# raphiniert-com/volume_renderer

Hardware: AMD Instinct MI355X
Metric: Mrays/s + achieved HBM GB/s, 1024³ vol @ 1920×1080 HG-shaded, 1/2/4/8 GPU (higher is better)
Workload: dtype f32; 1 GPU; V_shell(1024) fp32 1024^3, 1920x1080, HG 2 lights (example1.m), on-the-fly gradient, rotate(125,25,0) f=3 dist=6 thr=0.9; lights=2, gradient=compute, parallelism=image-column partition x1 (block 16), depth_lanes=2, frames=serial, one HIP stream

## Files before the change

volume_renderer_amd/csrc/vr_capi.hip:

```cpp
#include <hip/hip_runtime.h>

#include <algorithm>
#include <chrono>
#include <cmath>
#include <cstdio>
#include <cstdlib>
#include <cstring>
#include <memory>
#include <mutex>
#include <map>
#include <set>
#include <array>
#include <sstream>
#include <string>
#include <queue>
#include <vector>

#include "../../include/vrhip.h"
#include "vr_device.h"
#include "vr_resources.h"
#include "vr_transfer.h"

#ifndef VR_WITH_K8
#define VR_WITH_K8 0
// ... 361 lines not shown
  if (!want || b->occ_bytes != bytes) {
    if (b->occ) vr_host::pooled_free(b->occ, b->occ_bytes, b->device, vr_host::Readers(b->readers));
    b->occ = nullptr;
    b->occ_bytes = 0;
  }
  if (!want) return;
  if (!b->occ) {
    VR_HIP(vr_host::pooled_alloc(reinterpret_cast<void **>(&b->occ), bytes, b->device));
    b->occ_bytes = bytes;
  }
  const float inv = (!b->nonfinite && b->maxabs > 0.f) ? 255.f / b->maxabs : 0.f;
  VR_HIP(vr::launch_occupancy(b->ptr, (uint32_t)px, (uint32_t)py, (uint32_t)pz, b->occ, std::isfinite(inv) ? inv : 0.f,
                              s));
  VR_HIP(hipStreamSynchronize(s));
}

void sync_volume(vr_context *h, int tex, int slot) {
  g_tex.bind[tex].reset();
  const VolRec &v = h->vol[slot];
  const uint64_t n = v.dims[0] * v.dims[1] * v.dims[2];
  const uint64_t padded = n ? (v.dims[0] + 2) * (v.dims[1] + 2) * (v.dims[2] + 2) * sizeof(float) : 0;
  BufPtr b = h->buf[slot];
  if (!(b && b.use_count() == 2 && b->bytes == padded && b->device == h->device && b->readers.done())) {
    h->buf[slot].reset();
    b = std::make_shared<DevBuf>();
    b->device = h->device;
    b->bytes = padded;
    if (padded) VR_HIP(vr_host::pooled_alloc(reinterpret_cast<void **>(&b->ptr), padded, h->device));
  }
  for (int i = 0; i < 3; ++i) b->dims[i] = v.dims[i];
  b->nonfinite = false;
  b->maxabs = 0.f;
  b->readers.clear();
  if (n) {
    if (!v.data) throw HipError{hipErrorInvalidValue, "volume data is NULL"};
    vr_host::Uploader &U = vr_host::uploaders()[h->device];
    VR_HIP(U.init(h->device));
    vr::BufStats st{0u, 0.f};
    VR_HIP(U.upload(v.data, v.dtype, v.location == VR_DEVICE, (int32_t)v.dims[0], (int32_t)v.dims[1],
                    (int32_t)v.dims[2], b->ptr, &st));
    b->nonfinite = st.nonfinite != 0;
    b->maxabs = st.maxabs;
    if (tex == T_LIGHT) build_zpair(b.get(), U.stream);
    else if (tex <= T_RE) build_occupancy(b.get(), U.stream);
  } else {
    build_occupancy(b.get(), nullptr);
  }
  b->version = next_version();
  b->src_data = v.data;
  b->src_last_update = v.last_update;
  b->src_bytes = v.memory_size;
  b->src_dtype = v.dtype;
  h->buf[slot] = b;
  g_tex.bind[tex] = b;
}

void sync_volume_if_changed(vr_context *h, int tex, int slot) {
  const BufPtr &b = g_tex.bind[tex];
  const VolRec &v = h->vol[slot];
  if (b && h->buf[slot] == b && b->device == h->device && v.data && b->src_data == v.data &&
      b->src_last_update == v.last_update && b->src_bytes == v.memory_size && b->src_dtype == v.dtype &&
      v.last_update != 0 &&
      !env_flag("VR_ALWAYS_REUPLOAD"))
    return;
  sync_volume(h, tex, slot);
}

template <class S>
void sync_decisions(S &s, bool simEmAb, bool simEmRe, bool simAbRe, bool reqEm, bool reqAb, bool reqRe) {
  bool updEm = false, updAb = false, updRe = false;
  if (reqEm) {
    if (!updEm) { s.upload(T_EM); updEm = true; }
    if (simEmRe && !updRe) { s.reference(T_RE, T_RE, &S::idx_re, T_EM); updRe = true; }
    if (simEmAb && !updAb) { s.reference(T_AB, T_AB, &S::idx_ab, T_EM); updAb = true; }
  }
  if (reqAb) {
    if (!updAb) { s.upload(T_AB); updAb = true; }
    if (simAbRe && !updRe) { s.reference(T_RE, T_RE, &S::idx_re, T_AB); updRe = true; }
    if (simEmAb && !updEm) { s.reference(T_EM, T_AB, &S::idx_em, T_AB); updEm = true; }
  }
  if (reqRe) {
    if (!updRe) { s.upload(T_RE); updRe = true; }
    if (simAbRe && !updAb) { s.reference(T_AB, T_AB, &S::idx_ab, T_RE); updAb = true; }
    if (simEmAb && !updEm) { s.reference(T_EM, T_EM, &S::idx_em, T_RE); updEm = true; }
  }
}

struct RealState {
  vr_context *h;
  int32_t idx_em, idx_ab, idx_re;
  void upload(int slot) { sync_volume(h, slot, slot); }
  void reference(int tex, int bufslot, int32_t RealState::*idx, int target) {
    if (h->buf[bufslot]) {
      g_tex.bind[tex].reset();
      h->buf[bufslot].reset();
    }
    this->*idx = target;
  }
};

struct DebugState {
  bool present[3] = {true, true, true};
  bool bound[3] = {true, true, true};
  int32_t idx_em, idx_ab, idx_re;
  void upload(int slot) { present[slot] = true; bound[slot] = true; }
  void reference(int tex, int bufslot, int32_t DebugState::*idx, int target) {
    if (present[bufslot]) {
      bound[tex] = false;
      present[bufslot] = false;
    }
    this->*idx = target;
  }
};

uint64_t required_memory(const vr_context *h) {
  const VolRec &em = h->vol[T_EM], &ab = h->vol[T_AB], &re = h->vol[T_RE];
  uint64_t r = em.memory_size;
  if (!same(em, ab) && !same(re, ab)) r += ab.memory_size;
  if (!same(em, re) && !same(re, ab)) r += re.memory_size;
  r += h->vol[T_DX].memory_size + h->vol[T_DY].memory_size + h->vol[T_DZ].memory_size;
  return r;
}

int check_free_device_memory(uint64_t required) {
  size_t free_b = 0, total_b = 0;
  VR_HIP(hipMemGetInfo(&free_b, &total_b));
  if (free_b >= required) return VR_OK;
  int dev = 0;
  VR_HIP(hipGetDevice(&dev));
  vr_host::pool_clear(dev);
  vr_host::prune_retired(true);
  VR_HIP(hipMemGetInfo(&free_b, &total_b));
  if (free_b >= required) return VR_OK;
  std::ostringstream os;
  os << "insufficient free VRAM!\n"
     << "\tTotal Memory (MB): \t" << total_b / (1024 * 1024) << "\n"
     << "\tFree Memory (MB): \t" << free_b / (1024 * 1024) << "\n"
     << "\tRequired memory (MB): \t" << required / (1024 * 1024) << "\n";
  return fail(VR_ERR_VRAM, os.str());
}

void reset_gradients(vr_context *h) {
  for (int s : {T_DX, T_DY, T_DZ}) {
    h->buf[s].reset();
    h->vol[s] = VolRec();
  }
}

void mm_sync(vr_context *h) {
  if ((h->vol[T_DX].last_update == 0 && h->buf[T_DX]) || (h->vol[T_DY].last_update == 0 && h->buf[T_DY]) ||
      (h->vol[T_DZ].last_update == 0 && h->buf[T_DZ]))
    reset_gradients(h);
  const VolRec &em = h->vol[T_EM], &ab = h->vol[T_AB], &re = h->vol[T_RE];
  const uint64_t T = h->time_last_mem_sync;
  RealState s{h, g_tex.idx_em, g_tex.idx_ab, g_tex.idx_re};
  sync_decisions(s, same(em, ab), same(em, re), same(ab, re), em.last_update > T || T == 0,
                 ab.last_update > T || T == 0, re.last_update > T || T == 0);
  g_tex.idx_em = s.idx_em;
  g_tex.idx_ab = s.idx_ab;
  g_tex.idx_re = s.idx_re;
  if (h->vol[T_DX].last_update != 0 && h->vol[T_DY].last_update != 0 && h->vol[T_DZ].last_update != 0) {
    sync_volume_if_changed(h, T_DX, T_DX);
    sync_volume_if_changed(h, T_DY, T_DY);
    sync_volume_if_changed(h, T_DZ, T_DZ);
    g_tex.grad_method = G_LOOKUP;
  }
}

vr::DevTex dev_tex(const BufPtr &b) {
  vr::DevTex t{};
  if (b && b->ptr) {
    t.p = b->ptr;
    t.nx = (int32_t)b->dims[0];
    t.ny = (int32_t)b->dims[1];
    t.nz = (int32_t)b->dims[2];
    t.px = (uint32_t)(b->dims[0] + 2);
    t.pxy = (uint32_t)((b->dims[0] + 2) * (b->dims[1] + 2));
    t.fnx = (float)t.nx;
    t.fny = (float)t.ny;
    t.fnz = (float)t.nz;
    t.one = (t.nx == 1 && t.ny == 1 && t.nz == 1);
    const uint64_t padded = (b->dims[0] + 2) * (b->dims[1] + 2) * (b->dims[2] + 2);
    t.small = padded < (1ull << 22) && !test_flag("VR_NO_SMALL_LUT");
    t.fpx4 = 4.f * (float)t.px;
    t.fpxy4 = 4.f * (float)t.pxy;
    t.fbase4 = 4.f * (float)(t.pxy + t.px + 1);
    t.zp = t.small ? b->zpair : nullptr;
  }
  return t;
}

bool is_big(const vr::DevTex &t) {
  return t.p && ((uint64_t)t.nx + 2) * ((uint64_t)t.ny + 2) * ((uint64_t)t.nz + 2) > 0xFFFFFFFFull;
}

bool same_tex(const vr::DevTex &a, const vr::DevTex &b) {
  return a.p == b.p && a.nx == b.nx && a.ny == b.ny && a.nz == b.nz;
}
bool same_dims(const vr::DevTex &a, const vr::DevTex &b) {
  return a.nx == b.nx && a.ny == b.ny && a.nz == b.nz;
}

bool tame(const BufPtr &b) { return !b || !b->ptr || (!b->nonfinite && b->maxabs < 1e30f); }

int32_t half_texel_taps(const vr::RenderParams &P, int mode, float fnz) {
  if (mode != 1 || test_flag("VR_EXACT_TAPS")) return 0;
  const float n[3] = {P.em.fnx, P.em.fny, fnz};
  for (int i = 0; i < 3; ++i) {
    int e = 0;
    if (!(n[i] >= 2.f) || std::frexp(n[i], &e) != 0.5f) return 0;
    if (P.gstep[i] != 1.f / n[i] || P.bscale[i] != 0.5f || P.bmin[i] != -1.f) return 0;
  }
  return 1;
}

struct Frame {
  vr::RenderParams P;
  double drift1[3] = {0, 0, 0};
  int mode = 0;
  bool ab_alias = false, big = false, share = false;
  bool degenerate = false;
  vr_context::Schedule *sched_copy = nullptr;
  vr_context::Schedule *sched = nullptr;
};


void drift_bound(Frame &F, const float *eye2) {
  const vr::RenderParams &P = F.P;
  double pmax = 0.0;
  for (int i = 0; i < 3; ++i) {
    double e = std::fabs(P.eye[i]);
    if (eye2) e = std::max(e, (double)std::fabs(eye2[i]));
    pmax = std::max(pmax, (double)std::fabs(P.bmin[i]) + e);
  }
  for (int i = 0; i < 3; ++i) {
    const float n = i == 0 ? P.em.fnx : (i == 1 ? P.em.fny : P.em.fnz);
    F.drift1[i] = 2.0 * pmax * 1.2e-7 * (double)P.bscale[i] * (double)n;
    F.P.probe_off[i] = (float)(0.0625 + (double)VR_PROBE_MAX * F.drift1[i]);
  }
}

int build_frame(vr_context *h, const vr_render_args *a, Frame &F, uint64_t depth_override = 0) {
  vr::RenderParams &P = F.P;
  std::memset(&P, 0, sizeof(P));
  const uint64_t H = a->resolution[0], W = a->resolution[1];
  if (W > 0x7FFFFFFF || H > 0x7FFFFFFF || W * H > (1ull << 40))
    return fail(VR_ERR_UNSUPPORTED, "image resolution too large");
  P.width = (int32_t)W;
  P.height = (int32_t)H;
  P.fw = (float)W;
  P.fh = (float)H;
  P.ratio = (float)H / (float)W;
  P.fe = a->factors[0];
  P.fr = a->factors[1];
  P.fa = a->factors[2];
  const float es[3] = {a->element_size_um[2], a->element_size_um[1], a->element_size_um[0]};
  const VolRec &ev = h->vol[T_EM];
  const uint64_t vw = ev.dims[0], vh = ev.dims[1], vd = depth_override ? depth_override : ev.dims[2];
  float bmax[3];
  bmax[0] = 1.f;
  bmax[1] = (es[1] * (float)vh) / ((float)vw * es[0]);
  bmax[2] = (es[2] * (float)vd) / ((float)vw * es[0]);
  for (int i = 0; i < 3; ++i) P.bmin[i] = -1.f * bmax[i];
  const float dxy = sqrtf((float)(vw * vw + vh * vh));
  const float dyz = sqrtf((float)(vh * vh + vd * vd));
  const float dxz = sqrtf((float)(vw * vw + vd * vd));
  const float mind = fminf(dxy, fminf(dyz, dxz));
  P.tstep = 1.f / (2.2f * mind);
  P.thr = a->opacity_threshold;
  for (int i = 0; i < 3; ++i) {
    P.bscale[i] = 1.f / (bmax[i] - P.bmin[i]);
    P.color[i] = a->color[i];
  }
  P.gstep[0] = 1.f / (float)vw;
  P.gstep[1] = 1.f / (float)vh;
  P.gstep[2] = 1.f / (float)vd;
  const float *r = a->rotation_flipped;
  const float X[3] = {r[2], r[1], r[0]}, Y[3] = {r[5], r[4], r[3]}, Z[3] = {r[8], r[7], r[6]};
  const float xoff = a->props[0], f = a->props[1], dist = a->props[2];
  for (int i = 0; i < 3; ++i) {
    P.eye[i] = fmaf(-dist, Z[i], xoff * X[i]);
    P.ydir[i] = Y[i];
    P.zdir[i] = Z[i];
  }
  const float xx = fmaf(X[2], X[2], fmaf(X[1], X[1], X[0] * X[0]));
  const float xinv = 1.f / sqrtf(xx);
  for (int i = 0; i < 3; ++i) P.nx_[i] = X[i] * xinv;
  P.focal = f;
  P.em = dev_tex(g_tex.bind[g_tex.idx_em]);
  {
    const BufPtr &eb = g_tex.bind[g_tex.idx_em];
    P.occ = (eb && eb->ptr && eb->occ) ? eb->occ : nullptr;
    constexpr uint64_t E = 1u << VR_OCC_LOG;
    P.occ_bx = P.occ ? (uint32_t)((eb->dims[0] + 2 + E - 1) / E) : 0u;
    P.occ_bxy = P.occ ? P.occ_bx * (uint32_t)((eb->dims[1] + 2 + E - 1) / E) : 0u;
  }
  P.ab = dev_tex(g_tex.bind[g_tex.idx_ab]);
  P.re = dev_tex(g_tex.bind[g_tex.idx_re]);
  P.gem = dev_tex(g_tex.bind[T_EM]);
  P.gx = dev_tex(g_tex.bind[T_DX]);
  P.gy = dev_tex(g_tex.bind[T_DY]);
  P.gz = dev_tex(g_tex.bind[T_DZ]);
  P.lut = dev_tex(g_tex.bind[T_LIGHT]);
  P.num_lights = (int32_t)g_tex.lights.size();
  P.lights = nullptr;
  F.mode = P.num_lights == 0 ? 0 : (g_tex.grad_method == G_LOOKUP ? 2 : 1);
  F.ab_alias = same_tex(P.ab, P.em);
  const bool em_grid = P.em.p && !P.em.one;
  if (F.mode == 1)
    F.share = em_grid && same_tex(P.gem, P.em);
  else if (F.mode == 2)
    F.share = em_grid && P.gx.p && P.gy.p && P.gz.p && !P.gx.one && same_dims(P.gx, P.em) &&
              same_dims(P.gy, P.em) && same_dims(P.gz, P.em);
  P.re_is_em = same_tex(P.re, P.em) && P.em.p != nullptr;
  {
    drift_bound(F, nullptr);
    for (int i = 0; i < 3; ++i) {
      const float n = i == 0 ? P.em.fnx : (i == 1 ? P.em.fny : P.em.fnz);
      P.tap_off[i] = (float)((F.mode == 1 ? (double)P.gstep[i] * P.bscale[i] * n : 0.0) + 0.0625);
    }
    P.tap_half = half_texel_taps(P, F.mode, P.em.fnz);
    P.cube_hs[0] = P.tap_half ? P.em.fnx * 0.5f : 0.f;
    P.cube_hs[1] = P.tap_half ? P.em.fny * 0.5f : 0.f;
    P.cube_hs[2] = P.tap_half ? P.em.fnz * 0.5f : 0.f;
  }
  {
    const BufPtr &rb = g_tex.bind[g_tex.idx_re];
    const BufPtr &lb = g_tex.bind[T_LIGHT];
    bool ok = tame(rb) && tame(lb) && std::isfinite(P.fr) && std::fabs(P.fr) < 1e3f;
    double bound = 1.0;
    for (int i = 0; i < 3; ++i) {
      ok = ok && std::isfinite(P.color[i]) && std::fabs(P.color[i]) < 1e3f;
      bound = std::max(bound, (double)std::fabs(P.color[i]));
    }
    double lmax = 0.0;
    for (const auto &L : g_tex.lights) {
      for (float c : {L.cr, L.cg, L.cb}) {
        ok = ok && std::isfinite(c);
        lmax = std::max(lmax, (double)std::fabs(c));
      }
    }
    const double rmax = (rb && rb->ptr) ? rb->maxabs : 0.0, lutmax = (lb && lb->ptr) ? lb->maxabs : 0.0;
    ok = ok && (double)std::fabs(P.fr) * rmax * lutmax * lmax * bound * (double)(g_tex.lights.size() + 1) < 1e36;
    P.skip_empty = ok ? 1 : 0;
    if (const char *ev = test_env("VR_NO_EMPTY_SKIP"))
      if (ev[0] == '1') P.skip_empty = 0;
    if (P.skip_empty && test_flag("VR_NO_BRICK_TEST")) P.skip_empty = 2;
  }
  {
    const BufPtr &eb = g_tex.bind[g_tex.idx_em], &ab = g_tex.bind[g_tex.idx_ab];
    auto vmax = [](const BufPtr &b) { return (b && b->ptr) ? (b->nonfinite ? INFINITY : (double)b->maxabs) : 0.0; };
    const double xa = std::fabs((double)P.fa) * vmax(ab) * (double)P.tstep;
    const double xe = std::fabs((double)P.fe) * vmax(eb) * (double)P.tstep;
    P.small_x = (std::isfinite(xa) && xa < 0x1p-7 * 0.999) ? 1 : 0;
    P.eds_finite = (std::isfinite(xe) && xe < 1e38) ? 1 : 0;
    if (diag_flag("VR_NO_RANGE_FLAGS")) P.small_x = P.eds_finite = 0;
  }
  {
    const bool re_ok = P.re_is_em || (P.re.p && P.re.one);
    const bool lut_ok = g_tex.lights.empty() || (P.lut.p && P.lut.small && !P.lut.one && P.lut.zp &&
                                                 std::max(P.lut.nx, std::max(P.lut.ny, P.lut.nz)) <= 8192);
    const bool step_ok = std::isfinite(P.tstep) && P.tstep > 0.f;
    P.tame = (P.skip_empty && P.eds_finite && P.small_x && re_ok && lut_ok && step_ok && !diag_flag("VR_NO_TAME")) ? 1
                                                                                                            : 0;
    P.re_mask = P.re_is_em ? 0xffffffffu : 0u;
  }
  F.big = is_big(P.em) || is_big(P.ab) || is_big(P.re) || is_big(P.gem) || is_big(P.gx) || is_big(P.gy) ||
          is_big(P.gz) || test_flag("VR_FORCE_BIG");
  if (F.mode == 2 && P.gx.p &&
      vr::interleave3_entries(P.gx.px, P.gx.pxy / P.gx.px, (uint32_t)P.gx.nz + 2u) > 0xFFFFFFFFull)
    F.big = true;
  if (is_big(P.lut)) return fail(VR_ERR_UNSUPPORTED, "illumination volume larger than 2^32 voxels");
  bool finite = std::isfinite(P.tstep) && P.tstep > 0.f;
  for (int i = 0; i < 3; ++i) finite = finite && std::isfinite(P.bmin[i]) && std::isfinite(P.bscale[i]);
  const double diag = std::sqrt(4.0 * ((double)bmax[0] * bmax[0] + (double)bmax[1] * bmax[1] +
                                       (double)bmax[2] * bmax[2]));
  const double cap = 2.0 * diag / (double)P.tstep + 64.0;
  P.max_steps = (finite && cap < 2.0e9) ? (int32_t)cap : 2000000000;
  F.degenerate = !finite;
  return VR_OK;
}

void upload_lights(vr_context *h, const vr_render_args *a) {
  if (a->num_lights < 0 || !a->illumination) return;
  const size_t n = (size_t)a->num_lights;
  g_tex.lights.resize(n);
  for (size_t l = 0; l < n; ++l) {
    const vr_light &L = a->lights[l];
    g_tex.lights[l] = vr::DevLight{L.position[2], L.position[1], L.position[0], L.color[0], L.color[1],
                                   L.color[2]};
  }
  h->vol[T_LIGHT] = make_rec(a->illumination);
  sync_volume_if_changed(h, T_LIGHT, T_LIGHT);
}

using LaunchRec = vr_host::LaunchRec<BufPtr>;
void wait_ready(const BufPtr &b, hipStream_t s) {
  if (b && !vr_host::done(b->ready)) VR_HIP(hipStreamWaitEvent(s, b->ready->e, 0));
}
void bind_reads(LaunchRec &L) {
  for (const BufPtr &b : g_tex.bind)
    if (b) {
      wait_ready(b, L.stream);
      L.reads.push_back(b);
    }
  for (const auto &kv : g_tex.gvec)
    if (kv.second.buf && kv.first == L.device) {
      wait_ready(kv.second.buf, L.stream);
      L.reads.push_back(kv.second.buf);
    }
}
void stage_frame(LaunchRec &L, vr::RenderParams &P, const std::vector<vr::DevLight> &lights) {
  const void *d = nullptr;
  VR_HIP(L.stage(lights.data(), lights.size() * sizeof(vr::DevLight), &d));
  P.lights = static_cast<const vr::DevLight *>(d);
}

int64_t part_columns(int64_t w, int32_t bc, int32_t part, int32_t np) {
  if (w <= 0) return 0;
  if (np <= 1) return w;
  const int64_t nblocks = (w + bc - 1) / bc;
  int64_t cols = 0;
  for (int64_t b = part; b < nblocks; b += np) cols += std::min<int64_t>(bc, w - b * bc);
  return cols;
}

int validate_partition(const vr_partition *p) {
  if (!p) return VR_OK;
  if (p->num_parts < 1 || p->part < 0 || p->part >= p->num_parts || p->block_cols < 1)
    return fail(VR_ERR_ARGUMENT, "invalid partition");
  return VR_OK;
}


int chunk_samples(int K) { return K >= 2 ? 16 * K : 32; }
void set_chunk_halo(Frame &F, int K) {
  for (int i = 0; i < 3; ++i) {
    F.P.tap_off[i] += (float)(chunk_samples(K) * F.drift1[i]);
  }
}

void free_views(vr_context *h) {
  if (h->d_chan) (void)hipFree(h->d_chan);
  h->d_chan = nullptr;
  h->d_chan_bytes = 0;
}

void free_schedules(vr_context *h) {
  for (auto &kv : h->sched) {
    if (kv.second.copied) (void)hipEventSynchronize(kv.second.copied);
    if (kv.second.d_cost) (void)hipFree(kv.second.d_cost);
    if (kv.second.d_order) (void)hipFree(kv.second.d_order);
    if (kv.second.h_cost) (void)hipHostFree(kv.second.h_cost);
    if (kv.second.pre_flag) (void)hipFree(kv.second.pre_flag);
    if (kv.second.pre_count) (void)hipFree(kv.second.pre_count);
    if (kv.second.pre_state) (void)hipFree(kv.second.pre_state);
    if (kv.second.copied) (void)hipEventDestroy(kv.second.copied);
  }
  h->sched.clear();
}

int device_wave_slots() {
  static int slots = 0;
  if (!slots) {
    int dev = 0, cus = 256;
    if (hipGetDevice(&dev) == hipSuccess) {
      hipDeviceProp_t prop;
      if (hipGetDeviceProperties(&prop, dev) == hipSuccess && prop.multiProcessorCount > 0)
        cus = prop.multiProcessorCount;
    }
    slots = cus * 16;
  }
  return slots;
}

#ifndef VR_COUNT_K
#define VR_COUNT_K 0
#endif
#ifndef VR_XCD_RUN
#define VR_XCD_RUN 0
#endif

int depth_lanes(const vr::RenderParams &P) {
  if (const char *ev = test_env("VR_DEPTH_LANES")) {
    const int k = std::atoi(ev);
    if (k == 1 || k == 2 || k == 4 || (k == 8 && VR_WITH_K8)) return k;
  }
  const double waves = std::ceil(P.part_cols / 8.0) * std::ceil(P.height / 8.0);
  const double rounds = waves / device_wave_slots();
  const double tau = P.tau > 0.f ? (double)P.tau : 1.0;
  if (P.lookup) return 4;
  if (rounds < VR_DEPTH_ROUNDS_K2 || tau >= VR_DEPTH_TAU_K4) return 4;
  if (rounds >= VR_DEPTH_ROUNDS_K1 && tau < VR_DEPTH_TAU_K1) return 1;
  return 2;
}

void set_tau_and_slot(vr::RenderParams &P, const vr_render_args *a, double vw) {
  const double f = std::fabs((double)a->props[1]), dist = std::fabs((double)a->props[2]);
  const double tau = (f > 0 && P.width > 0) ? dist * vw / ((double)P.width * f) : 1e30;
  P.tau = (float)std::min(tau, 1e30);
  const int K = P.steps ? 1 : depth_lanes(P);
  P.wide_slot = (tau > 1.5 || (K >= 4 && !P.lookup)) ? 1 : 0;
  if (const char *ev = test_env("VR_WIDE_SLOT")) P.wide_slot = std::atoi(ev) ? 1 : 0;
}

bool short_launch(const vr::RenderParams &P) {
  const double rounds = std::ceil(P.part_cols / 8.0) * std::ceil(P.height / 8.0) * std::max(1, (int)P.views) /
                        device_wave_slots();
  return rounds < VR_SCHED_ROUNDS;
}
#ifndef VR_SCHED_LPT_ROUNDS
#define VR_SCHED_LPT_ROUNDS 32.0
#endif
bool lpt_launch(const vr::RenderParams &P) {
  const double rounds = std::ceil(P.part_cols / 8.0) * std::ceil(P.height / 8.0) * std::max(1, (int)P.views) /
                        device_wave_slots();
  return rounds < VR_SCHED_ROUNDS || rounds >= VR_SCHED_LPT_ROUNDS;
}
bool want_schedule(const vr::RenderParams &P) {
  if (P.views > 2 || (P.views == 2 && test_flag("VR_STEREO_PAIR")) || test_flag_off("VR_SCHED")) return false;
  return test_flag("VR_SCHED") || short_launch(P) || !test_flag_off("VR_SCHED_FULL");
}

uint64_t wg_tail_arg(uint32_t tail_pct) {
  return (uint64_t)tail_pct << 32 | (uint64_t)(device_wave_slots() / 16 * 6);
}

uint64_t frame_key(const vr::RenderParams &P) {
  uint64_t h = 1469598103934665603ull;
  auto mix = [&h](const void *p, size_t n) {
    const unsigned char *c = static_cast<const unsigned char *>(p);
    for (size_t i = 0; i < n; ++i) h = (h ^ c[i]) * 1099511628211ull;
  };
  mix(P.eye, sizeof P.eye);
  mix(P.eye2, sizeof P.eye2);
  mix(P.nx_, sizeof P.nx_);
  mix(P.ydir, sizeof P.ydir);
  mix(P.zdir, sizeof P.zdir);
  mix(&P.focal, sizeof P.focal);
  mix(P.bmin, sizeof P.bmin);
  mix(&P.tstep, sizeof P.tstep);
  mix(&P.thr, sizeof P.thr);
  mix(&P.fa, sizeof P.fa);
  mix(&P.fe, sizeof P.fe);
  mix(&P.em.p, sizeof P.em.p);
  mix(&P.occ, sizeof P.occ);
  const BufPtr &eb = g_tex.bind[g_tex.idx_em];
  const uint64_t ver = (eb && eb->ptr == P.em.p) ? eb->version : 0;
  mix(&ver, sizeof ver);
  return h | 1u;
}

#ifndef VR_PRED_STEP_TEXELS
#define VR_PRED_STEP_TEXELS 8.0
#endif
hipError_t predict_costs(const vr::RenderParams &P, int K, uint32_t nb_view, uint32_t *cost, hipStream_t stream) {
  const int TW = K == 1 ? 8 : (K == 2 ? 4 : (K == 4 ? 4 : 2)), TH = K <= 2 ? 8 : 4;
  const uint32_t nbx = (uint32_t)((P.part_cols + 2 * TW - 1) / (2 * TW));
  const BufPtr &eb = g_tex.bind[g_tex.idx_em];
  double dens = 0.0;
  if (eb && !eb->nonfinite && P.fa > 0.f && std::isfinite(P.fa))
    dens = (double)P.fa * (double)eb->maxabs / 255.0 * (double)P.tstep;
  const double xthr = P.thr < 1.f ? -std::log1p(-(double)std::max(P.thr, 0.f)) : 1e30;
  double tpa = 0.0;
  for (int i = 0; i < 3; ++i) {
    const float n = i == 0 ? P.em.fnx : (i == 1 ? P.em.fny : P.em.fnz);
    tpa = std::max(tpa, (double)P.bscale[i] * (double)n);
  }
  const double per = (double)P.tstep * tpa;
  const int m = (int)std::max(1.0, std::min(4096.0, std::floor(VR_PRED_STEP_TEXELS / std::max(per, 1e-9))));
  const hipError_t rc = vr::launch_predict_cost(P, nb_view, nbx, TW, TH, m, (float)dens, (float)std::min(xthr, 1e30),
                                                cost, stream);
  if (const char *dump = rc == hipSuccess ? diag_env("VR_SCHED_PRED_DUMP") : nullptr) {
    const uint32_t nb = nb_view * (uint32_t)std::max(1, (int)P.views);
    std::vector<uint32_t> c(nb);
    VR_HIP(hipMemcpyAsync(c.data(), cost, (size_t)nb * 4, hipMemcpyDeviceToHost, stream));
    VR_HIP(hipStreamSynchronize(stream));
    const uint32_t hdr[4] = {(uint32_t)K, (uint32_t)P.part, (uint32_t)P.num_parts, nb};
    if (FILE *f = std::fopen(dump, "ab")) {
      std::fwrite(hdr, 4, 4, f);
      std::fwrite(c.data(), 4, c.size(), f);
      std::fclose(f);
    }
  }
  return rc;
}

hipError_t attach_schedule(vr_context *h, vr::RenderParams &P, Frame &F, int K, hipStream_t stream,
                           const char *extra) {
  typedef uint32_t (*blocks_fn)(const vr::RenderParams &);
  static const blocks_fn bfns[4] = {vr::fast::march_blocks_k1, vr::fast::march_blocks_k2, vr::fast::march_blocks_k4,
                                    VR_K8(vr::fast::march_blocks_k8, vr::fast::march_blocks_k4)};
  const int ki = K == 1 ? 0 : K == 2 ? 1 : K == 4 ? 2 : 3;
  const uint32_t nb_view = bfns[ki](P);
  const uint32_t nb = nb_view * (uint32_t)std::max(1, (int)P.views);
  char key[300];
  std::snprintf(key, sizeof key, "%d/%d/%d/%d/%d/%d/%d/%d/%d/%u/%p/%s", K, P.width, P.height, P.part, P.num_parts,
                P.block_cols, F.mode, P.wide_slot, P.fast_shade, nb, (void *)stream, extra);
  vr_context::Schedule &S = h->sched[key];
  F.sched = &S;
  if (!S.d_cost && nb) {
    hipError_t e = hipMalloc(&S.d_cost, nb * sizeof(uint32_t));
    if (e == hipSuccess) e = hipMalloc(&S.d_order, nb * sizeof(uint32_t));
    if (e != hipSuccess) {
      vr_host::consume(e, "hipMalloc (launch schedule; the launch runs unscheduled)");
      if (S.d_cost) (void)hipFree(S.d_cost);
      S.d_cost = nullptr;
      S.d_order = nullptr;
    }
    S.blocks = nb;
  }
  if (!(S.d_cost && S.blocks == nb)) return hipSuccess;
  hipError_t rc = hipSuccess;
  const bool full = !lpt_launch(P) && !test_flag("VR_SCHED");
  const uint64_t fkey = frame_key(P);
  const bool predict = P.occ && P.occ_bx && !diag_flag("VR_SCHED_MEASURED");
  if (!full) {
    P.sched_full = 0;
    if (S.measured && S.key == fkey) {
      rc = vr::launch_order(S.d_cost, nb, S.d_order, stream, 0u, 0u);
    } else if (predict) {
      rc = predict_costs(P, K, nb_view, S.d_cost, stream);
      if (rc == hipSuccess) rc = vr::launch_order(S.d_cost, nb, S.d_order, stream, 0u, 0u);
    } else {
      rc = vr::launch_iota(S.d_order, nb, stream);
    }
    S.measured = true;
    S.key = fkey;
    S.pred_key = 0;
  } else {
    if (S.key != fkey) {
      if (S.copy_pending) {
        (void)hipEventSynchronize(S.copied);
        S.copy_pending = false;
      }
      S.measured = S.decided = S.tail = S.order_stale = false;
      S.frames = S.renders = 0;
      S.key = fkey;
    }
    ++S.renders;
    uint32_t every = VR_SCHED_REMEASURE;
    if (const char *ev = test_env("VR_SCHED_REMEASURE")) every = (uint32_t)std::max(1, std::atoi(ev));
    uint32_t heavy_div = VR_SCHED_HEAVY_DIV;
    if (const char *ev = diag_env("VR_SCHED_HEAVY_DIV")) heavy_div = (uint32_t)std::max(1, std::atoi(ev));
    uint32_t tail_pct = VR_SCHED_TAIL_PCT;
    if (const char *ev = test_env("VR_SCHED_TAIL_PCT")) tail_pct = (uint32_t)std::max(0, std::atoi(ev));
    if (!S.h_cost) {
      hipError_t e = hipHostMalloc(reinterpret_cast<void **>(&S.h_cost), nb * sizeof(uint32_t));
      if (e == hipSuccess) e = hipEventCreateWithFlags(&S.copied, hipEventDisableTiming);
      if (e != hipSuccess) {
        vr_host::consume(e, "hipHostMalloc / hipEventCreate (full-frame schedule; none used)");
        return hipSuccess;
      }
    }
    if (S.copy_pending && vr_host::query_done(S.copied, "hipEventQuery (schedule durations)")) {
      S.copy_pending = false;
      uint64_t sum = 0;
      uint32_t mx = 0;
      for (uint32_t i = 0; i < nb; ++i) {
        sum += S.h_cost[i];
        mx = std::max(mx, S.h_cost[i]);
      }
      const uint64_t wg_slots = std::max<uint64_t>(1, (uint64_t)(device_wave_slots() / 16 * 6));
      S.tail = (uint64_t)mx * 100u >= (sum / wg_slots) * tail_pct;
      S.decided = true;
      S.order_stale = true;
    }
    if (predict && !S.decided) {
      if (S.pred_key != fkey) {
        rc = predict_costs(P, K, nb_view, S.d_cost, stream);
        if (rc == hipSuccess) rc = vr::launch_order(S.d_cost, nb, S.d_order, stream, heavy_div, wg_tail_arg(0));
        S.pred_key = rc == hipSuccess ? fkey : 0;
      }
      if (S.renders >= 2 && !S.measured && !diag_flag("VR_SCHED_PREDICT_ONLY")) {
        S.measured = true;
        S.frames = 0;
        P.sched_full = 1;
        F.sched_copy = &S;
      } else {
        P.sched_full = 2;
      }
// ... 1914 lines not shown
```

volume_renderer_amd/csrc/vr_device.h:

```cpp
#pragma once
#include <stdint.h>
#include <hip/hip_runtime.h>

namespace vr {

struct DevTex {
  const float *p;
  int32_t nx, ny, nz;
  uint32_t px;
  uint32_t pxy;
  float fnx, fny, fnz;
  int32_t one;
  int32_t small;
  float fpx4, fpxy4, fbase4;
  const float *zp;
};

#ifndef VR_PROBE_MAX
#define VR_PROBE_MAX 512
#endif

#ifndef VR_OCC_LOG
#define VR_OCC_LOG 3
#endif

#ifndef VR_GVEC_BRICK
#define VR_GVEC_BRICK 1
#endif

struct DevLight {
  float px, py, pz;
  float cr, cg, cb;
};

struct RenderParams {
  int32_t width, height;
  float fw, fh;
  float ratio;
  float fe, fa, fr;
  float bmin[3];
  float bscale[3];
  float eye[3];
  float eye2[3];
  float nx_[3];
  float ydir[3], zdir[3];
  float focal;
  float thr, tstep;
  int32_t max_steps;
  float color[3];
  float gstep[3];
  float tap_off[3];
  int32_t tap_half;
  float cube_hs[3];
  int32_t num_lights;
  const DevLight *lights;
  DevTex em, ab, re, gem, gx, gy, gz, lut;
  const float *gvec;
  uint32_t gv_row8, gv_plane8;
  int32_t re_is_em;
  int32_t skip_empty;
  int32_t small_x;
  int32_t eds_finite;
  int32_t tame;
  uint32_t re_mask;
  float tau;
  int32_t lookup;
  int32_t tile_mode;
  int32_t xcd_run;
  uint32_t block_rot;
  int32_t wide_slot;
  int32_t fast_shade;
  int32_t block_cols, part, num_parts, part_cols;
  int32_t plane_cols;
  float *out;
  float *out2;
  int32_t views;
  int32_t pair_shift;
  uint32_t view_blocks;
  const uint32_t *wg_order;
  uint32_t *wg_cost;
  uint32_t *wg_start;
  uint32_t sched_blocks;
  uint32_t sched_full;
  uint32_t prio_blocks;
  const uint8_t *occ;
  uint32_t occ_bx, occ_bxy;
  float probe_off[3];
  unsigned long long *steps;
  float slab_z0, slab_z1, slab_margin;
  int32_t slab_pk0, slab_pk1, slab_dir;
  const float *slab_in;
  const uint32_t *pre_flag;
  float4 *pre_state;
  uint32_t *pre_count;
  uint32_t pre_cap;
};

#define VR_VIEWS_MAX 4
struct RenderViews {
  RenderParams p[VR_VIEWS_MAX];
};
static_assert(sizeof(RenderViews) <= 4160, "RenderParams grew: RenderViews passes four by value as kernel arguments");

struct BufStats {
  uint32_t nonfinite;
  float maxabs;
};

void note_march_kernel(bool fast, int K, int mode, bool ab, bool count, bool share, bool big, int cap, int sched,
                       int nl);
bool test_switches_on();

}
```

volume_renderer_amd/csrc/vr_march.hip:

```cpp
#include <hip/hip_runtime.h>
#include <stdint.h>
#include <math.h>
#include <stdlib.h>
#include <algorithm>
#include <type_traits>

#ifndef VR_MARCH_K
#define VR_MARCH_K 1
#endif
#ifndef VR_MERGED_BOUNDS
#define VR_MERGED_BOUNDS 1
#endif
#ifndef VR_WHOLE_BOX
#define VR_WHOLE_BOX 1
#endif
#ifndef VR_CHECK_WHOLE
#define VR_CHECK_WHOLE 0
#endif
#ifndef VR_LIGHTS_HOIST
#define VR_LIGHTS_HOIST 1
#endif
#ifndef VR_REFL_HOIST
#define VR_REFL_HOIST 1
#endif
#ifndef VR_ADAPTIVE_S
#define VR_ADAPTIVE_S 1
#endif
#ifndef VR_WHOLE_SPLIT
#define VR_WHOLE_SPLIT 1
#endif
#ifndef VR_COUNT_K
#define VR_COUNT_K 0
#endif
#if VR_CHECK_WHOLE
static __device__ unsigned long long vr_whole_violations;
#endif
#ifndef VR_BRANCHFREE_LEAP
#define VR_BRANCHFREE_LEAP 1
#endif
#ifndef VR_CHUNK_PER_LANE
#define VR_CHUNK_PER_LANE 16
#endif
#ifndef VR_CHUNK
#define VR_CHUNK (VR_MARCH_K >= 2 ? VR_CHUNK_PER_LANE * VR_MARCH_K : 32)
#endif
static_assert(VR_CHUNK <= (VR_MARCH_K >= 2 ? 16 * VR_MARCH_K : 32), "chunk longer than the host's halo margin");

#include "vr_device.h"
#include "vr_sampling.h"
#include "vr_stage.h"

namespace vr {

#ifndef VR_MARCH_FAST
#define VR_MARCH_FAST 1
#endif
#if VR_MARCH_FAST
namespace fast {
#else
namespace exact {
#endif

#define VR_CAT2(a, b) a##b
#define VR_CAT(a, b) VR_CAT2(a, b)

template <int K, int I>
__device__ __forceinline__ float group_lane(float v) {
  if constexpr (K == 1) {
    return v;
  } else if constexpr (K == 2) {
    constexpr int ctrl = I | (I << 2) | ((2 + I) << 4) | ((2 + I) << 6);
    return __int_as_float(__builtin_amdgcn_mov_dpp(__float_as_int(v), ctrl, 0xf, 0xf, true));
  } else if constexpr (K == 4) {
    constexpr int ctrl = I | (I << 2) | (I << 4) | (I << 6);
    return __int_as_float(__builtin_amdgcn_mov_dpp(__float_as_int(v), ctrl, 0xf, 0xf, true));
  } else {
    static_assert(K == 8, "depth lanes: K in {1, 2, 4, 8}");
    return __int_as_float(__builtin_amdgcn_ds_swizzle(__float_as_int(v), 0x18 | (I << 5)));
  }
}

struct Ray {
  f3 o, pos, step;
  float t, tfar;
  float sr, sg, sb, sa;
  int32_t nsteps, nlit;
  bool alive;
  bool mine;
  bool past;
};

__device__ __forceinline__ void store_resume(const RenderParams &P, uint32_t kk, float t, const f3 &pos, int32_t n) {
  const size_t plane = (size_t)P.plane_cols * (size_t)P.height;
  P.out[kk + 5 * plane] = t;
  P.out[kk + 6 * plane] = pos.x;
  P.out[kk + 7 * plane] = pos.y;
  P.out[kk + 8 * plane] = pos.z;
  P.out[kk + 9 * plane] = __int_as_float(n);
}

template <int K, int I = K - 1>
__device__ __forceinline__ void first_of_group(float flagf, float t0, const f3 &p0, int32_t n0, float &t, f3 &p,
                                               int32_t &n) {
  if constexpr (I >= 0) {
    const float x = group_lane<K, I>(p0.x), y = group_lane<K, I>(p0.y), z = group_lane<K, I>(p0.z);
    const float tt = group_lane<K, I>(t0);
    const int32_t nn = __float_as_int(group_lane<K, I>(__int_as_float(n0)));
    if (group_lane<K, I>(flagf) != 0.f) {
      t = tt;
      p = mk(x, y, z);
      n = nn;
    }
    first_of_group<K, I - 1>(flagf, t0, p0, n0, t, p, n);
  }
}

struct ChunkStats {
  uint32_t staged, leap, fall, iter, lit, probe, probe_fail;
};

#ifndef VR_CUBE_AXIS
#define VR_CUBE_AXIS 1
#endif
#ifndef VR_PROBE
#define VR_PROBE 1
#endif
#ifndef VR_NL2
#define VR_NL2 1
#endif
#ifndef VR_PARK
#define VR_PARK 1
#endif
#ifndef VR_PARK_SAMPLES
#define VR_PARK_SAMPLES (2 * VR_CHUNK)
#endif
#ifndef VR_REPROBE_PARTIAL
#define VR_REPROBE_PARTIAL 1
#endif
#ifndef VR_PRELEAP
#define VR_PRELEAP 1
#endif
#ifndef VR_PRELEAP_SPREAD
#define VR_PRELEAP_SPREAD 256
#endif
#ifndef VR_PROBE_LANES
#define VR_PROBE_LANES 0
#endif
#ifndef VR_PROBE_BISECT
#define VR_PROBE_BISECT 1
#endif
#ifndef VR_PROBE_MIN
#define VR_PROBE_MIN (2 * VR_CHUNK)
#endif

template <int MODE, bool AB_ALIAS, bool SHARE2, bool BIG, bool NANCHK, int NL = 0>
__device__ __forceinline__ void sample_at(const RenderParams &P, const float *L, const Box &B, bool staged, bool whole,
                                          const f3 pos, const f3 o, float &r, float &gg, float &b, float &alpha,
                                          bool &shaded, float rv = 0.f, const DevLight *pre = nullptr) {
  const DevTex &E = P.em;
  const f3 bmin = mk(P.bmin[0], P.bmin[1], P.bmin[2]);
  const f3 bsc = mk(P.bscale[0], P.bscale[1], P.bscale[2]);
  const float tstep = P.tstep;
  const f3 ps = mk((pos.x - bmin.x) * bsc.x, (pos.y - bmin.y) * bsc.y, (pos.z - bmin.z) * bsc.z);
  constexpr bool HALF_TAPS = VR_MARCH_FAST && MODE == 1;
  constexpr bool HALF_ONLY = HALF_TAPS && SHARE2;
  AxS sx{}, sy{}, sz{};
  Ax ax, ay, az;
  if constexpr (HALF_ONLY && VR_CUBE_AXIS) {
    sx = axis_cube_s<NANCHK>(pos.x, P.cube_hs[0]);
    sy = axis_cube_s<NANCHK>(pos.y, P.cube_hs[1]);
    sz = axis_cube_s<NANCHK>(pos.z, P.cube_hs[2]);
    ax = Ax{sx.i, sx.w};
    ay = Ax{sy.i, sy.w};
    az = Ax{sz.i, sz.w};
  } else if constexpr (HALF_TAPS) {
    sx = axis_raw_s<NANCHK>(ps.x, E.fnx);
    sy = axis_raw_s<NANCHK>(ps.y, E.fny);
    sz = axis_raw_s<NANCHK>(ps.z, E.fnz);
    ax = Ax{sx.i, sx.w};
    ay = Ax{sy.i, sy.w};
    az = Ax{sz.i, sz.w};
  } else {
    ax = axis_raw<NANCHK>(ps.x, E.fnx);
    ay = axis_raw<NANCHK>(ps.y, E.fny);
    az = axis_raw<NANCHK>(ps.z, E.fnz);
  }
  const int lx = slot_coord(ax.i, B.rx), ly = slot_coord(ay.i, B.ry), lz = slot_coord(az.i, B.rz);
#define inx in_box(lx, B.ex)
#define iny in_box(ly, B.ey)
#define inz in_box(lz, B.ez)
  const int ayz = lz * B.pxy + ly * B.px;
  const int ac = ayz + lx;
  Cell C;
  float em_s;
  bool full = false;
  if constexpr (HALF_ONLY && VR_MERGED_BOUNDS) {
    if (VR_WHOLE_BOX && !VR_CHECK_WHOLE && whole) {
      full = true;
    } else {
      full = __all(staged && (unsigned)(lx + (sx.hi ? 1 : 0) - 1) < (unsigned)(B.ex - 2) &&
                   (unsigned)(ly + (sy.hi ? 1 : 0) - 1) < (unsigned)(B.ey - 2) &&
                   (unsigned)(lz + (sz.hi ? 1 : 0) - 1) < (unsigned)(B.ez - 2));
#if VR_CHECK_WHOLE
      if (whole && !full && __lane_id() == __builtin_amdgcn_readfirstlane(__lane_id())) {
        const unsigned long long c = atomicAdd(&vr_whole_violations, 1ull);
        if (c < 8 || c % 100000 == 0)
          printf("VR_CHECK_WHOLE: whole box misses a tap (#%llu): cell %d %d %d box %d %d %d + %d %d %d\n", c, ax.i,
                 ay.i, az.i, B.rx, B.ry, B.rz, B.ex, B.ey, B.ez);
      }
#endif
    }
  }
  if constexpr (HALF_TAPS) {
    if (full) em_s = lds_tri_cell(L, B, ac, ax.w, ay.w, az.w, C);
    else if (staged && inx && iny && inz) em_s = lds_tri_cell(L, B, ac, ax.w, ay.w, az.w, C);
    else {
      const DevTex U = reload(E);
      em_s = fetch<BIG>(U, clamp_ax(ax, U.nx), clamp_ax(ay, U.ny), clamp_ax(az, U.nz));
    }
  } else {
    em_s = fetch_at<BIG>(E, L, B, staged && inx && iny && inz, ac, ax, ay, az);
  }
  const float ab_s = AB_ALIAS ? em_s : tex3d<BIG>(P.ab, ps.x, ps.y, ps.z);
  const float e = P.fe * em_s;
  const float a = P.fa * ab_s;
  constexpr bool TAME = !NANCHK;
  if constexpr (TAME) alpha = opacity<VR_MARCH_FAST>(a, tstep, true);
  else alpha = P.small_x ? opacity<VR_MARCH_FAST>(a, tstep, true) : opacity<VR_MARCH_FAST>(a, tstep);
  const float eds = e * tstep;
  float ir = 0.f, ig = 0.f, ib = 0.f;
  const bool skip = TAME ? alpha == 0.f : (P.skip_empty && alpha == 0.f && (P.eds_finite || fabsf(eds) <= 3.0e38f));
  shaded = MODE != 0 && !skip;
  if (MODE != 0 && !skip) {
    f3 g;
    if ((MODE == 1 && (VR_ABLATE & 4)) || (MODE == 2 && (VR_ABLATE & 32))) {
      g = mk(ps.x, ps.y, em_s);
    } else if (HALF_TAPS && (HALF_ONLY || P.tap_half) &&
               (full || __all(staged && (unsigned)(lx + (sx.hi ? 1 : 0) - 1) < (unsigned)(B.ex - 2) &&
                     (unsigned)(ly + (sy.hi ? 1 : 0) - 1) < (unsigned)(B.ey - 2) &&
                     (unsigned)(lz + (sz.hi ? 1 : 0) - 1) < (unsigned)(B.ez - 2)))) {
      g = half_grad_lds(L, B, ac, sx, sy, sz, ax.w, ay.w, az.w, C);
    } else if (HALF_TAPS && (HALF_ONLY || P.tap_half)) {
      const bool syz = staged && iny && inz, sxz = staged && inx && inz, sxy = staged && inx && iny;
      Ax p, m;
      half_taps(sx, p, m);
      int l = lx + (sx.hi ? 1 : 0);
      int a = ac + (sx.hi ? 1 : 0);
      g.x = fetch_at<BIG>(E, L, B, syz && in_box(l, B.ex), a, p, ay, az) -
            fetch_at<BIG>(E, L, B, syz && in_box(l - 1, B.ex), a - 1, m, ay, az);
      half_taps(sy, p, m);
      l = ly + (sy.hi ? 1 : 0);
      a = ac + (sy.hi ? B.px : 0);
      g.y = fetch_at<BIG>(E, L, B, sxz && in_box(l, B.ey), a, ax, p, az) -
            fetch_at<BIG>(E, L, B, sxz && in_box(l - 1, B.ey), a - B.px, ax, m, az);
      half_taps(sz, p, m);
      l = lz + (sz.hi ? 1 : 0);
      a = ac + (sz.hi ? B.pxy : 0);
      g.z = fetch_at<BIG>(E, L, B, sxy && in_box(l, B.ez), a, ax, ay, p) -
            fetch_at<BIG>(E, L, B, sxy && in_box(l - 1, B.ez), a - B.pxy, ax, ay, m);
    } else if (MODE == 1) {
      const float xp = ((pos.x + P.gstep[0]) - bmin.x) * bsc.x;
      const float xm = ((pos.x - P.gstep[0]) - bmin.x) * bsc.x;
      const float yp = ((pos.y + P.gstep[1]) - bmin.y) * bsc.y;
      const float ym = ((pos.y - P.gstep[1]) - bmin.y) * bsc.y;
      const float zp = ((pos.z + P.gstep[2]) - bmin.z) * bsc.z;
      const float zm = ((pos.z - P.gstep[2]) - bmin.z) * bsc.z;
      const bool syz = staged && iny && inz, sxz = staged && inx && inz, sxy = staged && inx && iny;
      const Ax axp = axis_raw<NANCHK>(xp, E.fnx), axm = axis_raw<NANCHK>(xm, E.fnx);
      const int lxp = slot_coord(axp.i, B.rx), lxm = slot_coord(axm.i, B.rx);
      g.x = fetch_at<BIG>(E, L, B, syz && in_box(lxp, B.ex), ayz + lxp, axp, ay, az) -
            fetch_at<BIG>(E, L, B, syz && in_box(lxm, B.ex), ayz + lxm, axm, ay, az);
      const Ax ayp = axis_raw<NANCHK>(yp, E.fny), aym = axis_raw<NANCHK>(ym, E.fny);
      const int lyp = slot_coord(ayp.i, B.ry), lym = slot_coord(aym.i, B.ry);
      const int axz = lz * B.pxy + lx;
      g.y = fetch_at<BIG>(E, L, B, sxz && in_box(lyp, B.ey), axz + lyp * B.px, ax, ayp, az) -
            fetch_at<BIG>(E, L, B, sxz && in_box(lym, B.ey), axz + lym * B.px, ax, aym, az);
      const Ax azp = axis_raw<NANCHK>(zp, E.fnz), azm = axis_raw<NANCHK>(zm, E.fnz);
      const int lzp = slot_coord(azp.i, B.rz), lzm = slot_coord(azm.i, B.rz);
      const int axy = ly * B.px + lx;
      g.z = fetch_at<BIG>(E, L, B, sxy && in_box(lzp, B.ez), axy + lzp * B.pxy, ax, ay, azp) -
            fetch_at<BIG>(E, L, B, sxy && in_box(lzm, B.ez), axy + lzm * B.pxy, ax, ay, azm);
      g = mk(g.x * 0.5f, g.y * 0.5f, g.z * 0.5f);
    } else if (MODE == 2 && SHARE2) {
      const Ax cx = clamp_ax(ax, E.nx), cy = clamp_ax(ay, E.ny), cz = clamp_ax(az, E.nz);
      if (P.gvec)
        g = fetch_vec<BIG>(P.gvec, P.gx, P.gv_row8, P.gv_plane8, cx, cy, cz);
      else
        g = mk(fetch<BIG>(P.gx, cx, cy, cz), fetch<BIG>(P.gy, cx, cy, cz), fetch<BIG>(P.gz, cx, cy, cz));
    } else {
      g = mk(tex3d<BIG>(P.gx, ps.x, ps.y, ps.z), tex3d<BIG>(P.gy, ps.x, ps.y, ps.z),
             tex3d<BIG>(P.gz, ps.x, ps.y, ps.z));
    }
    float refl;
    if constexpr (TAME) {
      const float v = VR_REFL_HOIST ? rv : voxel0(P.re.p);
      const uint32_t m = P.re_mask;
      refl = P.fr * __uint_as_float((__float_as_uint(em_s) & m) | (__float_as_uint(fmaf(0.5f, v - v, v)) & ~m));
    } else {
      refl = P.fr * (P.re_is_em ? em_s : tex3d<BIG>(P.re, ps.x, ps.y, ps.z));
    }
    shade_lights<VR_MARCH_FAST, TAME, NL>(P, g, pos, o, refl, ir, ig, ib, pre);
  }
  r = fmaf(eds, P.color[0], ir) * alpha;
  gg = fmaf(eds, P.color[1], ig) * alpha;
  b = fmaf(eds, P.color[2], ib) * alpha;
#undef inx
#undef iny
#undef inz
}

__device__ __forceinline__ void composite(const RenderParams &P, Ray &R, float r, float gg, float b, float alpha,
                                          float thr, int cap) {
  const float om = 1.f - R.sa;
  R.sr = fmaf(om, r, R.sr);
  R.sg = fmaf(om, gg, R.sg);
  R.sb = fmaf(om, b, R.sb);
  R.sa = fmaf(om, alpha, R.sa);
  ++R.nsteps;
  if (R.sa > thr || R.nsteps >= cap) {
    R.alive = false;
  } else {
    R.t += P.tstep;
    if (R.t > R.tfar) R.alive = false;
    else R.pos = mk(R.pos.x + R.step.x, R.pos.y + R.step.y, R.pos.z + R.step.z);
  }
}

#ifndef VR_GROUP_ANY_DPP
#define VR_GROUP_ANY_DPP 1
#endif
template <int K>
__device__ __forceinline__ bool group_any(bool b) {
  if constexpr ((K == 2 || K == 4) && VR_GROUP_ANY_DPP) {
    int v = b ? 1 : 0;
    v |= __builtin_amdgcn_mov_dpp(v, 0xB1, 0xf, 0xf, true);
    if constexpr (K == 4) v |= __builtin_amdgcn_mov_dpp(v, 0x4E, 0xf, 0xf, true);
    return v != 0;
  } else {
    const uint64_t m = __ballot(b);
    const int base = (int)(__lane_id() & ~(uint32_t)(K - 1));
    return ((m >> base) & ((1ull << K) - 1)) != 0ull;
  }
}

template <int K, int I = 0>
__device__ __forceinline__ int group_max_i(int v, int acc) {
  if constexpr (K == 1 || I == K) {
    return acc;
  } else {
    return group_max_i<K, I + 1>(v, max(acc, __float_as_int(group_lane<K, I>(__int_as_float(v)))));
  }
}

#ifndef VR_ZERO_FILL
#define VR_ZERO_FILL 1
#endif
template <int K, int I, bool ZF = false>
__device__ __forceinline__ void composite_group(const RenderParams &P, Ray &R, float exf, float r, float gg, float b,
                                                float alpha, float thr) {
  if constexpr (K == 2 && ZF && I < K) {
    if (R.alive) {
      const float om = 1.f - R.sa;
      if constexpr (I == 0)
        asm("s_nop 1\n\t"
            "v_fmac_f32_dpp %0, %4, %8 quad_perm:[0,0,2,2] row_mask:0xf bank_mask:0xf\n\t"
            "v_fmac_f32_dpp %1, %5, %8 quad_perm:[0,0,2,2] row_mask:0xf bank_mask:0xf\n\t"
            "v_fmac_f32_dpp %2, %6, %8 quad_perm:[0,0,2,2] row_mask:0xf bank_mask:0xf\n\t"
            "v_fmac_f32_dpp %3, %7, %8 quad_perm:[0,0,2,2] row_mask:0xf bank_mask:0xf"
            : "+v"(R.sr), "+v"(R.sg), "+v"(R.sb), "+v"(R.sa)
            : "v"(r), "v"(gg), "v"(b), "v"(alpha), "v"(om));
      else
        asm("s_nop 1\n\t"
            "v_fmac_f32_dpp %0, %4, %8 quad_perm:[1,1,3,3] row_mask:0xf bank_mask:0xf\n\t"
            "v_fmac_f32_dpp %1, %5, %8 quad_perm:[1,1,3,3] row_mask:0xf bank_mask:0xf\n\t"
            "v_fmac_f32_dpp %2, %6, %8 quad_perm:[1,1,3,3] row_mask:0xf bank_mask:0xf\n\t"
            "v_fmac_f32_dpp %3, %7, %8 quad_perm:[1,1,3,3] row_mask:0xf bank_mask:0xf"
            : "+v"(R.sr), "+v"(R.sg), "+v"(R.sb), "+v"(R.sa)
            : "v"(r), "v"(gg), "v"(b), "v"(alpha), "v"(om));
      if (R.sa > thr) R.alive = false;
    }
    composite_group<K, I + 1, ZF>(P, R, exf, r, gg, b, alpha, thr);
  } else if constexpr (I < K) {
    const float ri = group_lane<K, I>(r), gi = group_lane<K, I>(gg), bi = group_lane<K, I>(b),
                ai = group_lane<K, I>(alpha);
    if ((ZF || group_lane<K, I>(exf) != 0.f) && R.alive) {
      const float om = 1.f - R.sa;
      R.sr = fmaf(om, ri, R.sr);
      R.sg = fmaf(om, gi, R.sg);
      R.sb = fmaf(om, bi, R.sb);
      R.sa = fmaf(om, ai, R.sa);
      if (R.sa > thr) R.alive = false;
    }
    composite_group<K, I + 1, ZF>(P, R, exf, r, gg, b, alpha, thr);
  }
}

template <int K, int MODE, bool AB_ALIAS, bool COUNT, bool SHARE2, bool BIG, bool NANCHK, int CAP, bool SLAB = false,
          int NL = 0>
__device__ __forceinline__ void march(const RenderParams &P, float *L, int lane, Ray &R, ChunkStats &C,
                                      uint32_t kk = 0, KParams kp = nullptr, uint32_t gw = 0) {
  static_assert(!COUNT || K == 1 || VR_COUNT_K, "the counter variant is built for K = 1 only (VR_COUNT_K: all K)");
  static_assert(!SLAB || (!COUNT && BIG), "slab mode: no counters, 64-bit addressing");
  const int cap = P.max_steps;
  const float thr = P.thr;
  const float sbz = P.bmin[2], ssz = P.bscale[2];
  auto beyond = [&](float zn) { return R.step.z >= 0.f ? zn >= P.slab_z1 : zn < P.slab_z0; };
  const DevTex &E = P.em;
  const int sub = lane & (K - 1);
  if constexpr (K > 1) {
    R.mine = R.alive;
    leap(P, sub, R.mine, R.nsteps, R.t, R.tfar, R.pos, R.step, cap);
    R.alive = group_any<K>(R.mine);
  }

  int s0 = VR_CHUNK;
  constexpr bool PROBE = VR_PROBE && !NANCHK && AB_ALIAS && !SLAB;
  int ps = VR_PROBE_MIN;
  float rv = 0.f;
  if constexpr (!NANCHK && VR_REFL_HOIST) {
    if (P.tame && P.re.p) rv = voxel0(P.re.p);
    asm volatile("" : "+v"(rv));
  }
  DevLight pre2[2];
  const DevLight *pre = nullptr;
  if constexpr (!NANCHK && VR_LIGHTS_HOIST && MODE != 0 && K > 1 && AB_ALIAS && SHARE2 && !BIG && !SLAB && !COUNT) {
    const bool two = NL == 2 || (NL == 0 && P.num_lights >= 2);
    for (int j = 0; j < 2; ++j) {
      pre2[j] = (two || (NL == 1 && j == 0)) ? light_at(P, j) : DevLight{0.f, 0.f, 0.f, 0.f, 0.f, 0.f};
      asm volatile("" : "+v"(pre2[j].px), "+v"(pre2[j].py), "+v"(pre2[j].pz), "+v"(pre2[j].cr), "+v"(pre2[j].cg),
                   "+v"(pre2[j].cb));
    }
    if (two || NL == 1) pre = pre2;
  }
  auto leap_run = [&](int n) __attribute__((always_inline)) {
    if constexpr (K == 1) {
      if (COUNT || !VR_BRANCHFREE_LEAP) leap(P, n, R.alive, R.nsteps, R.t, R.tfar, R.pos, R.step, cap);
      else if constexpr (!NANCHK) advance_n(P, n, R.alive, R.nsteps, R.t, R.tfar, R.pos, R.step, cap);
      else advance(P, n, R.alive, R.nsteps, R.t, R.tfar, R.pos, R.step, cap);
    } else {
      if constexpr (!NANCHK) advance_n(P, n, R.mine, R.nsteps, R.t, R.tfar, R.pos, R.step, cap);
      else advance(P, n, R.mine, R.nsteps, R.t, R.tfar, R.pos, R.step, cap);
      R.alive = R.alive && group_any<K>(R.mine);
    }
  };
  if constexpr (PROBE && VR_PRELEAP && !COUNT) {
    if (kp != nullptr) {
      const KParams kq = kparams_fresh(kp);
      if (kq->pre_flag != nullptr) {
        const uint32_t f = __builtin_amdgcn_readfirstlane(kq->pre_flag[gw]);
        if (__builtin_expect(f != 0u, 0)) {
          const float4 *st = kq->pre_state + ((size_t)(f - 1u) * 64u + (uint32_t)lane) * 2u;
          const float4 a = st[0], b = st[1];
          R.t = a.x;
          R.pos = mk(a.y, a.z, a.w);
          R.nsteps = __float_as_int(b.x);
          const int fl = __float_as_int(b.y);
          R.alive = (fl & 1) != 0;
          R.mine = (fl & 2) != 0;
        }
      }
    }
  }
  while (__any(R.alive)) {
    if constexpr (PROBE) {
      if (ps > 0 && kp != nullptr && kparams_fresh(kp)->occ != nullptr) {
        const bool live = K > 1 ? (R.alive && R.mine) : R.alive;
        auto probe = [&](int len) __attribute__((always_inline)) {
          const int r = probe_run(P, kp, live, R.pos, R.step, R.t, R.tfar, len, lane);
          return (VR_PROBE_LANES && r < 0) ? probe_lanes(P, kp, live, R.pos, R.step, R.t, R.tfar, len) : r;
        };
        int e = probe(ps);
        while (VR_PROBE_BISECT && e <= 0 && ps > VR_PROBE_MIN) {
          ps >>= 1;
          e = probe(ps);
        }
        if (e > 0) {
          if (COUNT) ++C.probe;
          leap_run(ps);
          ps = min(2 * ps, (int)VR_PROBE_MAX);
          continue;
        }
        if (COUNT) ++C.probe_fail;
        ps = 0;
      }
    }
    int S;
    bool staged, partial;
    Box B;
    int box_vol = 0;
    bool edge = true;
    plan_chunk<CAP>(P, K > 1 ? (R.alive && R.mine) : R.alive, R.pos, R.step, R.t, R.tfar, S, staged, partial, B,
                    COUNT ? &box_vol : nullptr, &edge, s0);
    bool parked_any = false;
    if constexpr (VR_PARK && !SLAB && !NANCHK) {
      if (!staged || partial) {
        const bool lv = K > 1 ? (R.alive && R.mine) : R.alive;
        const int tmin = wave_min(lv ? __float_as_int(R.t) : 0x7f7fffff);
        bool pk = lv && R.t > __int_as_float(tmin) + (float)VR_PARK_SAMPLES * P.tstep;
        if constexpr (K > 1) pk = group_any<K>(pk);
        if (__any(pk)) {
          parked_any = true;
          if (pk) {
            R.alive = false;
            R.t = -R.t;
          }
          plan_chunk<CAP>(P, K > 1 ? (R.alive && R.mine) : R.alive, R.pos, R.step, R.t, R.tfar, S, staged, partial,
                          B, COUNT ? &box_vol : nullptr, &edge, s0);
        }
      }
    }
    auto unpark = [&]() __attribute__((always_inline)) {
      if (parked_any && __float_as_int(R.t) < 0) {
        R.t = -R.t;
        R.alive = true;
      }
    };
    if (VR_ADAPTIVE_S)
      s0 = (staged && !partial) ? min(2 * S, (int)VR_CHUNK) : (int)(VR_CHUNK >> (VR_ATTEMPTS - 1));
    bool inside = true;
    if constexpr (SLAB) {
      bool own = false, in = true;
      if (R.alive) {
        const float zs = (R.pos.z - sbz) * ssz;
        const float ze = (fmaf(R.step.z, (float)(S - 1), R.pos.z) - sbz) * ssz;
        own = fmaxf(zs, ze) + P.slab_margin >= P.slab_z0 && fminf(zs, ze) - P.slab_margin < P.slab_z1;
        in = fminf(zs, ze) - P.slab_margin >= P.slab_z0 && fmaxf(zs, ze) + P.slab_margin < P.slab_z1;
      }
      if (!__any(own)) staged = false;
      inside = __all(in);
      const int z_lo = max(B.rz, P.slab_pk0), z_hi = min(B.rz + B.ez, P.slab_pk1);
      if (staged) {
        if (z_hi - z_lo < 3) {
          staged = false;
        } else {
          B.rz = z_lo;
          B.ez = z_hi - z_lo;
        }
      }
    }
    bool empty = false;
    if constexpr (PROBE) {
      if (staged && !partial && ps == 0)
        empty = box_bricks_empty(kp, B.rx, B.ry, B.rz, B.ex, B.ey, B.ez, lane) > 0;
    }
    if (COUNT && lane == 0) {
      if (!staged || partial) atomicAdd(P.steps + 8 + min(box_vol >> 8, 31), 1ull);
      else atomicAdd(P.steps + 40 + (S >= 32 ? 0 : (S >= 16 ? 1 : (S >= 8 ? 2 : 3))), 1ull);
      if (staged && !empty) atomicAdd(P.steps + 45, (unsigned long long)(B.pxy * B.ez));
      if (empty) atomicAdd(P.steps + 46, 1ull);
    }
    if (staged && !empty) {
      const bool nonzero = stage_box<BIG>(L, E, B, lane);
      empty = AB_ALIAS && P.skip_empty && !partial && !nonzero && (!SLAB || inside);
    }
    __builtin_amdgcn_wave_barrier();
    if (COUNT) ++(staged && !partial ? (empty ? C.leap : C.staged) : C.fall);
    const bool whole = __builtin_amdgcn_readfirstlane((!NANCHK && !SLAB && staged && !partial && !edge) ? 1 : 0) != 0;

    if (empty) {
      if (!parked_any) leap_run(S);
      else if (__float_as_int(R.t) >= 0) leap_run(S);
      unpark();
      if (PROBE && ps < 0) ps = VR_PROBE_MIN;
      continue;
    }
    if (PROBE) ps = (VR_PROBE_LANES && VR_REPROBE_PARTIAL && partial) ? (int)VR_PROBE_MIN : -1;

    if constexpr (K == 1) {
      for (int k = 0; k < S && R.alive; ++k) {
        if (SLAB && !inside) {
          const float zn = (R.pos.z - sbz) * ssz;
          if (!(zn >= P.slab_z0 && zn < P.slab_z1)) {
            if (beyond(zn)) {
              store_resume(P, kk, R.t, R.pos, R.nsteps);
              R.alive = false;
              R.past = true;
            } else {
              ++R.nsteps;
              if (R.nsteps >= P.max_steps) {
                R.alive = false;
              } else {
                R.t += P.tstep;
                if (R.t > R.tfar) R.alive = false;
                else R.pos = mk(R.pos.x + R.step.x, R.pos.y + R.step.y, R.pos.z + R.step.z);
              }
            }
            continue;
          }
        }
        float r, gg, b, alpha;
        bool shaded;
        sample_at<MODE, AB_ALIAS, SHARE2, BIG, NANCHK, NL>(P, L, B, staged, whole, R.pos, R.o, r, gg, b, alpha, shaded,
                                                       rv, pre);
        if (COUNT) {
          ++C.iter;
          C.lit += (MODE != 0 && __any(shaded)) ? 1u : 0u;
          R.nlit += shaded ? 1 : 0;
        }
        composite(P, R, r, gg, b, alpha, thr, cap);
      }
    } else {
      auto samples = [&](auto wc) {
      constexpr bool WC = decltype(wc)::value;
      for (int k = 0, Su = __builtin_amdgcn_readfirstlane(S); k < Su; k += K) {
        if (!__any(R.alive)) break;
        if (!R.alive) continue;
        float r = 0.f, gg = 0.f, b = 0.f, alpha = 0.f;
        bool ex = R.mine, take = R.mine;
        if (SLAB && !inside) {
          const float zn = (R.pos.z - sbz) * ssz;
          if (ex && beyond(zn)) ex = false;
          take = ex && zn >= P.slab_z0 && zn < P.slab_z1;
        }
        bool shaded = false;
        if (take) {
          sample_at<MODE, AB_ALIAS, SHARE2, BIG, NANCHK, NL>(P, L, B, staged, WC || (!VR_WHOLE_SPLIT && whole), R.pos,
                                                         R.o, r, gg, b, alpha, shaded, rv, pre);
        }
        if (COUNT) {
          ++C.iter;
          C.lit += (MODE != 0 && __any(shaded)) ? 1u : 0u;
        }
        composite_group<K, 0, VR_ZERO_FILL && !NANCHK && !SLAB>(P, R, ex ? 1.f : 0.f, r, gg, b, alpha, thr);
        if (SLAB && !inside) {
          if (R.alive && group_any<K>(R.mine && !ex)) {
            float t = R.t;
            f3 p = R.pos;
            int32_t n = R.nsteps;
            first_of_group<K>((R.mine && !ex) ? 1.f : 0.f, R.t, R.pos, R.nsteps, t, p, n);
            if (sub == 0) store_resume(P, kk, t, p, n);
            R.alive = false;
            R.past = true;
          }
        }
        if constexpr (!NANCHK && !SLAB)
          advance_k<K>(P, R.mine, R.nsteps, R.t, R.tfar, R.pos, R.step, cap);
        else
          advance(P, K, R.mine, R.nsteps, R.t, R.tfar, R.pos, R.step, cap);
        R.alive = R.alive && group_any<K>(R.mine);
      }
      };
      if constexpr (VR_WHOLE_SPLIT && !NANCHK && !SLAB && VR_MARCH_FAST && MODE == 1 && SHARE2) {
        if (whole) samples(std::true_type{});
        else samples(std::false_type{});
      } else {
        samples(std::false_type{});
      }
    }
    unpark();
    __builtin_amdgcn_wave_barrier();
  }
}

__device__ __forceinline__ bool finite3(const f3 &v) {
  return fabsf(v.x) <= 3.4e38f && fabsf(v.y) <= 3.4e38f && fabsf(v.z) <= 3.4e38f;
}

#ifndef VR_MARCH_MIN_EU
#define VR_MARCH_MIN_EU 5
#endif
#ifndef VR_SCHED1_MIN_EU
#define VR_SCHED1_MIN_EU 1
#endif
constexpr int march_min_eu(int cap, int sched) {
  return cap <= VR_LDS_CAP_MARCH ? (sched != 1 ? VR_MARCH_MIN_EU : VR_SCHED1_MIN_EU) : 1;
}
#ifndef VR_WG_WAVES
#define VR_WG_WAVES 4
#endif

template <int K>
struct TileShape {
  static constexpr int LR = (K == 1 ? 6 : K == 2 ? 5 : K == 4 ? 4 : 3);
  static constexpr int LK = 6 - LR;
#ifndef VR_TILE_WLOG
#define VR_TILE_WLOG -1
#endif
  static constexpr int LW = (VR_TILE_WLOG >= 0 && VR_TILE_WLOG <= LR) ? VR_TILE_WLOG : LR / 2;
  static constexpr int TW = 1 << LW, TH = 1 << (LR - LW);
};

__device__ __forceinline__ uint32_t xcd_block(uint32_t b, uint32_t n, int run) {
  if (run <= 1) return b;
  const uint32_t R = (uint32_t)run, gs = 8u * R, g = b / gs;
  if ((g + 1) * gs > n) return b;
  const uint32_t r = b - g * gs;
  return g * gs + (r & 7u) * R + (r >> 3);
}

template <int K, int MODE, bool AB_ALIAS, bool COUNT, bool SHARE2, bool BIG, int CAP, int SCHED, int NL>
__global__ __launch_bounds__(64 * VR_WG_WAVES, march_min_eu(CAP, SCHED)) void march_kernel(const RenderParams P) {
  using TS = TileShape<K>;
  __shared__ float lds[VR_WG_WAVES][CAP];
  const int lane = threadIdx.x & 63, wave = threadIdx.x >> 6;
  float *L = lds[wave];
  constexpr bool ORDERED = SCHED >= 1 && SCHED <= 3;
  constexpr bool TIMED = SCHED == 1 || SCHED == 2;
  constexpr bool PAIRED = SCHED == 4;
  const uint64_t clk0 = TIMED ? __builtin_amdgcn_s_memrealtime() : 0;
  uint32_t wgo = ORDERED ? P.wg_order[blockIdx.x] : xcd_block(blockIdx.x, gridDim.x, P.xcd_run);
  if (!ORDERED && P.block_rot) {
    wgo += P.block_rot;
    if (wgo >= gridDim.x) wgo -= gridDim.x;
  }
  if (ORDERED && blockIdx.x < P.prio_blocks) __builtin_amdgcn_s_setprio(2);
  int view, lc, y;
  if constexpr (PAIRED) {
    constexpr int TH2 = TS::TH / 2, HR = (64 / K) / 2;
    const int tile = (int)wgo * VR_WG_WAVES + wave;
    const int nbx = (P.part_cols + P.pair_shift + 2 * TS::TW - 1) / (2 * TS::TW);
    const int blk = tile >> 2, quad = tile & 3;
    const int ray = lane >> TS::LK, rr = ray & (HR - 1);
    view = ray >= HR ? 0 : 1;
    const int xv = (blk % nbx) * (2 * TS::TW) + (quad & 1) * TS::TW + rr / TH2;
    y = (blk / nbx) * (2 * TH2) + (quad >> 1) * TH2 + rr % TH2;
    lc = view ? xv - P.pair_shift : xv;
  } else {
    view = (P.views > 1 && wgo >= P.view_blocks) ? 1 : 0;
    const uint32_t wg = view ? wgo - P.view_blocks : wgo;
    const int tile = (int)wg * VR_WG_WAVES + wave;
    const int nbx = (P.part_cols + 2 * TS::TW - 1) / (2 * TS::TW);
    const int blk = tile >> 2, quad = tile & 3;
    const int ray = lane >> TS::LK;
    lc = (blk % nbx) * (2 * TS::TW) + (quad & 1) * TS::TW + (ray / TS::TH);
    y = (blk / nbx) * (2 * TS::TH) + (quad >> 1) * TS::TH + (ray % TS::TH);
  }
  float *const out = view ? P.out2 : P.out;
  const bool active = (!PAIRED || lc >= 0) && (lc < P.part_cols) && (y < P.height);
  Ray R;
  R.o = mk(0.f, 0.f, 0.f);
  R.pos = R.o;
  R.step = R.o;
  R.t = 0.f;
  R.tfar = -1.f;
  R.sr = R.sg = R.sb = R.sa = 0.f;
  R.nsteps = R.nlit = 0;
  R.alive = false;
  ChunkStats C{0, 0, 0, 0, 0, 0, 0};
  if (active) {
    const int blk = lc / P.block_cols, within = lc - blk * P.block_cols;
    const int x = (P.part + blk * P.num_parts) * P.block_cols + within;
    f3 d;
    float tnear;
    R.alive = ray_setup(P, x, y, R.o, d, tnear, R.tfar, view);
    R.pos = mk(fmaf(d.x, tnear, R.o.x), fmaf(d.y, tnear, R.o.y), fmaf(d.z, tnear, R.o.z));
    R.step = mk(d.x * P.tstep, d.y * P.tstep, d.z * P.tstep);
    R.t = tnear;
  }
  if (P.tame && __all(!R.alive || (finite3(R.pos) && finite3(R.step))))
    march<K, MODE, AB_ALIAS, COUNT, SHARE2, BIG, false, CAP, false, NL>(
        P, L, lane, R, C, 0u, (KParams)__builtin_amdgcn_kernarg_segment_ptr(), wgo * VR_WG_WAVES + (uint32_t)wave);
  else
    march<K, MODE, AB_ALIAS, COUNT, SHARE2, BIG, true, CAP>(P, L, lane, R, C);

  if (active && (__lane_id() & (K - 1)) == 0) {
    const size_t plane = (size_t)P.plane_cols * (size_t)P.height;
    const size_t kk = (size_t)lc * (size_t)P.height + (size_t)y;
    out[kk] = R.sr;
    out[kk + plane] = R.sg;
    out[kk + 2 * plane] = R.sb;
  }
  if (TIMED) {
    __syncthreads();
    if (threadIdx.x == 0) {
      const uint64_t d = __builtin_amdgcn_s_memrealtime() - clk0;
      P.wg_cost[wgo] = d > 0xffffffffull ? 0xffffffffu : (uint32_t)d;
      if (P.wg_start) P.wg_start[wgo] = (uint32_t)clk0;
    }
  }
  if (COUNT) {
    unsigned long long s = K == 1 ? (unsigned long long)R.nsteps : 0ull, l = K == 1 ? (unsigned long long)R.nlit : 0ull;
#pragma unroll
    for (int off = 32; off > 0; off >>= 1) {
      s += __shfl_xor(s, off, 64);
      l += __shfl_xor(l, off, 64);
    }
    if (lane == 0 && s) atomicAdd(P.steps, s);
    if (lane == 0 && l) atomicAdd(P.steps + 1, l);
    if (lane == 0) {
      atomicAdd(P.steps + 2, (unsigned long long)C.staged);
      atomicAdd(P.steps + 3, (unsigned long long)C.leap);
      atomicAdd(P.steps + 4, (unsigned long long)C.fall);
      atomicAdd(P.steps + 5, (unsigned long long)C.iter);
      atomicAdd(P.steps + 6, (unsigned long long)C.lit);
      atomicAdd(P.steps + 7, (unsigned long long)C.probe);
      atomicAdd(P.steps + 44, (unsigned long long)C.probe_fail);
    }
  }
}

template <int K>
__global__ __launch_bounds__(64 * VR_WG_WAVES) void preleap_kernel(const RenderParams P) {
  using TS = TileShape<K>;
  const int lane = threadIdx.x & 63, wave = threadIdx.x >> 6;
  const uint32_t wgo = blockIdx.x;
  const uint32_t gw = wgo * VR_WG_WAVES + (uint32_t)wave;
  const int view = (P.views > 1 && wgo >= P.view_blocks) ? 1 : 0;
  const uint32_t wg = view ? wgo - P.view_blocks : wgo;
  const int tile = (int)wg * VR_WG_WAVES + wave;
  const int nbx = (P.part_cols + 2 * TS::TW - 1) / (2 * TS::TW);
  const int blk = tile >> 2, quad = tile & 3;
  const int ray = lane >> TS::LK;
  const int lc = (blk % nbx) * (2 * TS::TW) + (quad & 1) * TS::TW + (ray / TS::TH);
  const int y = (blk / nbx) * (2 * TS::TH) + (quad >> 1) * TS::TH + (ray % TS::TH);
  const bool active = lc < P.part_cols && y < P.height;
  Ray R;
  R.pos = mk(0.f, 0.f, 0.f);
  R.step = R.pos;
  R.t = 0.f;
  R.tfar = -1.f;
  R.nsteps = 0;
  R.alive = false;
  if (active) {
    const int pb = lc / P.block_cols, within = lc - pb * P.block_cols;
    const int x = (P.part + pb * P.num_parts) * P.block_cols + within;
    f3 o, d;
    float tnear;
    R.alive = ray_setup(P, x, y, o, d, tnear, R.tfar, view);
    R.pos = mk(fmaf(d.x, tnear, o.x), fmaf(d.y, tnear, o.y), fmaf(d.z, tnear, o.z));
    R.step = mk(d.x * P.tstep, d.y * P.tstep, d.z * P.tstep);
    R.t = tnear;
  }
  const int cap = P.max_steps;
  uint32_t flag = 0;
  if (P.tame && P.occ != nullptr && __all(!R.alive || (finite3(R.pos) && finite3(R.step)))) {
    if constexpr (K > 1) {
      R.mine = R.alive;
      leap(P, lane & (K - 1), R.mine, R.nsteps, R.t, R.tfar, R.pos, R.step, cap);
      R.alive = group_any<K>(R.mine);
    } else {
      R.mine = R.alive;
    }
    const bool lv0 = K > 1 ? (R.alive && R.mine) : R.alive;
    const int tmn = wave_min(lv0 ? __float_as_int(R.t) : 0x7f7fffff);
    const int tmx = wave_max(lv0 ? __float_as_int(R.t) : 0);
    if (__int_as_float(tmx) > __int_as_float(tmn) + (float)VR_PRELEAP_SPREAD * P.tstep) {
      const KParams kq = (KParams)__builtin_amdgcn_kernarg_segment_ptr();
      bool go = lv0;
      while (group_any<K>(go)) {
        uint32_t v = 0;
        if (go) {
          const float rem = (R.tfar - R.t) / P.tstep;
          const int s_eff = (rem < (float)VR_PROBE_MAX) ? max((int)rem + 2, 1) : (int)VR_PROBE_MAX;
          const float k = (float)(s_eff - 1);
          const f3 pe = mk(fmaf(R.step.x, k, R.pos.x), fmaf(R.step.y, k, R.pos.y), fmaf(R.step.z, k, R.pos.z));
          v = probe_lane_walk(P.occ, P.occ_bx, P.occ_bxy, ((R.pos.x - P.bmin[0]) * P.bscale[0]) * P.em.fnx - 0.5f,
                              ((R.pos.y - P.bmin[1]) * P.bscale[1]) * P.em.fny - 0.5f,
                              ((R.pos.z - P.bmin[2]) * P.bscale[2]) * P.em.fnz - 0.5f,
                              ((pe.x - P.bmin[0]) * P.bscale[0]) * P.em.fnx - 0.5f,
                              ((pe.y - P.bmin[1]) * P.bscale[1]) * P.em.fny - 0.5f,
                              ((pe.z - P.bmin[2]) * P.bscale[2]) * P.em.fnz - 0.5f, kq->probe_off[0],
                              kq->probe_off[1], kq->probe_off[2], P.em.nx, P.em.ny, P.em.nz);
        }
        const bool data = group_any<K>(v != 0u);
        if (go && !data) {
          if constexpr (K == 1) {
            advance_n(P, (int)VR_PROBE_MAX, R.alive, R.nsteps, R.t, R.tfar, R.pos, R.step, cap);
            go = R.alive;
          } else {
            advance_n(P, (int)VR_PROBE_MAX, R.mine, R.nsteps, R.t, R.tfar, R.pos, R.step, cap);
            go = group_any<K>(R.mine);
          }
        } else {
          go = false;
        }
      }
      if constexpr (K > 1) R.alive = R.alive && group_any<K>(R.mine);
      if constexpr (K == 1) R.mine = R.alive;
      uint32_t slot = 0;
      if (lane == 0) slot = atomicAdd(P.pre_count, 1u);
      slot = __builtin_amdgcn_readfirstlane(slot);
      if (slot < P.pre_cap) {
        float4 *st = P.pre_state + ((size_t)slot * 64u + (uint32_t)lane) * 2u;
        st[0] = make_float4(R.t, R.pos.x, R.pos.y, R.pos.z);
        st[1] = make_float4(__int_as_float(R.nsteps), __int_as_float((R.alive ? 1 : 0) | (R.mine ? 2 : 0)), 0.f, 0.f);
        flag = slot + 1u;
      }
    }
  }
  if (lane == 0) const_cast<uint32_t *>(P.pre_flag)[gw] = flag;
}

#if !VR_ISA_PROBE
hipError_t VR_CAT(launch_preleap_k, VR_MARCH_K)(const RenderParams &P, hipStream_t s) {
  constexpr int K = VR_MARCH_K;
  using TS = TileShape<K>;
  if (P.part_cols <= 0 || P.height <= 0) return hipSuccess;
  if (!P.pre_flag || !P.pre_state || !P.pre_count || P.pair_shift) return hipErrorInvalidValue;
  const uint64_t tiles = (uint64_t)((P.part_cols + 2 * TS::TW - 1) / (2 * TS::TW)) *
                         (uint64_t)((P.height + 2 * TS::TH - 1) / (2 * TS::TH)) * 4;
  const uint32_t per_view = (uint32_t)((tiles + VR_WG_WAVES - 1) / VR_WG_WAVES);
  hipLaunchKernelGGL(preleap_kernel<K>, dim3(per_view * (P.views > 1 ? 2u : 1u)), dim3(64 * VR_WG_WAVES), 0, s, P);
  return hipGetLastError();
}
#endif

#if VR_MARCH_K <= 4
template <int K, int MODE, bool AB_ALIAS, bool COUNT, bool SHARE2, bool BIG, int CAP>
__device__ __forceinline__ void march_tile(const RenderParams &P, float *L, int lane, int wave, uint32_t wg,
                                           int view, float *out, Ray &R, ChunkStats &C, KParams kp) {
  using TS = TileShape<K>;
  const int tile = (int)wg * VR_WG_WAVES + wave;
  const int nbx = (P.part_cols + 2 * TS::TW - 1) / (2 * TS::TW);
  const int blk = tile >> 2, quad = tile & 3;
  const int ray = lane >> TS::LK;
  const int lc = (blk % nbx) * (2 * TS::TW) + (quad & 1) * TS::TW + (ray / TS::TH);
  const int y = (blk / nbx) * (2 * TS::TH) + (quad >> 1) * TS::TH + (ray % TS::TH);
  const bool active = (lc < P.part_cols) && (y < P.height);
  R.o = mk(0.f, 0.f, 0.f);
  R.pos = R.o;
  R.step = R.o;
  R.t = 0.f;
  R.tfar = -1.f;
  R.sr = R.sg = R.sb = R.sa = 0.f;
  R.nsteps = R.nlit = 0;
  R.alive = false;
  if (active) {
    const int blk = lc / P.block_cols, within = lc - blk * P.block_cols;
    const int x = (P.part + blk * P.num_parts) * P.block_cols + within;
    f3 d;
    float tnear;
    R.alive = ray_setup(P, x, y, R.o, d, tnear, R.tfar, view);
    R.pos = mk(fmaf(d.x, tnear, R.o.x), fmaf(d.y, tnear, R.o.y), fmaf(d.z, tnear, R.o.z));
    R.step = mk(d.x * P.tstep, d.y * P.tstep, d.z * P.tstep);
    R.t = tnear;
  }
  if (P.tame && __all(!R.alive || (finite3(R.pos) && finite3(R.step))))
    march<K, MODE, AB_ALIAS, COUNT, SHARE2, BIG, false, CAP>(P, L, lane, R, C, 0u, kp);
  else
    march<K, MODE, AB_ALIAS, COUNT, SHARE2, BIG, true, CAP>(P, L, lane, R, C);

  if (active && (lane & (K - 1)) == 0) {
    const size_t plane = (size_t)P.plane_cols * (size_t)P.height;
    const size_t kk = (size_t)lc * (size_t)P.height + (size_t)y;
    out[kk] = R.sr;
    out[kk + plane] = R.sg;
    out[kk + 2 * plane] = R.sb;
  }
}

template <int K, int MODE, bool AB_ALIAS, int CAP>
__global__ __launch_bounds__(64 * VR_WG_WAVES, march_min_eu(CAP, false)) void march_views_kernel(
    const RenderViews V, uint32_t per_view) {
  __shared__ float lds[VR_WG_WAVES][CAP];
  const int lane = threadIdx.x & 63, wave = threadIdx.x >> 6;
  const uint32_t view = blockIdx.x / per_view;
  const RenderParams &P = V.p[view];
  Ray R;
  ChunkStats C{0, 0, 0, 0, 0, 0, 0};
  const KParams kp = (KParams)((const __attribute__((address_space(4))) char *)__builtin_amdgcn_kernarg_segment_ptr() +
                               (size_t)view * sizeof(RenderParams));
  march_tile<K, MODE, AB_ALIAS, false, false, false, CAP>(P, lds[wave], lane, wave, blockIdx.x - view * per_view, 0,
                                                          P.out, R, C, kp);
}

#if !VR_ISA_PROBE
hipError_t VR_CAT(launch_march_views_k, VR_MARCH_K)(const RenderViews &V, uint32_t nviews, int mode, bool ab_alias,
                                                   hipStream_t s) {
  constexpr int K = VR_MARCH_K;
  using TS = TileShape<K>;
  const RenderParams &P0 = V.p[0];
  if (nviews > VR_VIEWS_MAX) return hipErrorInvalidValue;
  if (P0.part_cols <= 0 || P0.height <= 0 || nviews == 0) return hipSuccess;
  if (mode > 1 || P0.steps || P0.wg_order) return hipErrorInvalidValue;
  for (uint32_t v = 1; v < nviews; ++v)
    if (V.p[v].part_cols != P0.part_cols || V.p[v].height != P0.height || V.p[v].wide_slot != P0.wide_slot)
      return hipErrorInvalidValue;
  const uint64_t tiles = (uint64_t)((P0.part_cols + 2 * TS::TW - 1) / (2 * TS::TW)) *
                         (uint64_t)((P0.height + 2 * TS::TH - 1) / (2 * TS::TH)) * 4;
  const uint32_t per_view = (uint32_t)((tiles + VR_WG_WAVES - 1) / VR_WG_WAVES);
  if ((uint64_t)per_view * nviews > 0x7fffffffull) return hipErrorInvalidValue;
  const dim3 grid(per_view * nviews), blk(64 * VR_WG_WAVES);
#define VR_VIEWS_LAUNCH(M, A)                                                                                    \
  do {                                                                                                           \
    if (P0.wide_slot)                                                                                            \
      hipLaunchKernelGGL((march_views_kernel<K, M, A, VR_LDS_CAP_WIDE>), grid, blk, 0, s, V, per_view);         \
    else                                                                                                         \
      hipLaunchKernelGGL((march_views_kernel<K, M, A, VR_LDS_CAP>), grid, blk, 0, s, V, per_view);              \
  } while (0)
  if (mode == 0) {
    if (ab_alias) VR_VIEWS_LAUNCH(0, true);
    else VR_VIEWS_LAUNCH(0, false);
  } else {
    if (ab_alias) VR_VIEWS_LAUNCH(1, true);
    else VR_VIEWS_LAUNCH(1, false);
  }
#undef VR_VIEWS_LAUNCH
  return hipGetLastError();
}

#endif
#ifndef VR_SLAB_MIN_EU
#define VR_SLAB_MIN_EU 6
#endif
template <int K, int MODE, bool SH, int CAP, bool SCHED>
__global__ __launch_bounds__(64 * VR_WG_WAVES, (CAP <= VR_LDS_CAP && !SCHED) ? VR_SLAB_MIN_EU : 1) void march_slab_kernel(
    const RenderParams P) {
// ... 233 lines not shown
```

volume_renderer_amd/csrc/vr_sampling.h:

```cpp
#pragma once
#include <hip/hip_runtime.h>
#include <stdint.h>
#include <math.h>

#include "vr_device.h"

namespace vr {

#define VR_PI ((float)3.14159265358979323846f)

struct f3 {
  float x, y, z;
};
__device__ __forceinline__ f3 mk(float x, float y, float z) { return f3{x, y, z}; }
__device__ __forceinline__ float dot3(f3 a, f3 b) { return fmaf(a.z, b.z, fmaf(a.y, b.y, a.x * b.x)); }

typedef float f2a4 __attribute__((ext_vector_type(2), aligned(4)));
typedef float f4a8 __attribute__((ext_vector_type(4), aligned(8)));

struct Ax {
  int i;
  float w;
};
__device__ __forceinline__ float weight8(float xb, float fl) {
  return fmaf(rintf(xb * 256.f), 1.f / 256.f, -fl);
}
#define VR_RN_MAGIC 49152.f
__device__ __forceinline__ float frac8_rn(float r) { return (r + VR_RN_MAGIC) - VR_RN_MAGIC; }
__device__ __forceinline__ float weight8_rn(float xb, float fl) { return ((xb + VR_RN_MAGIC) - VR_RN_MAGIC) - fl; }
template <bool NANCHK = true>
__device__ __forceinline__ Ax axis(float c, int n, float fn) {
  if (NANCHK) c = (c != c) ? 0.f : c;
  const float xb = c * fn - 0.5f;
  const float fl = floorf(xb);
  const float w = weight8(xb, fl);
  (void)n;
  return Ax{(int)__builtin_amdgcn_fmed3f(fl, -1.f, fn - 1.f), w};
}

template <bool NANCHK = true>
__device__ __forceinline__ Ax axis_raw(float c, float fn) {
  if (NANCHK) c = (c != c) ? 0.f : c;
  const float xb = c * fn - 0.5f;
  const float fl = floorf(xb);
  const float w = weight8(xb, fl);
  return Ax{(int)fl, w};
}
__device__ __forceinline__ Ax clamp_ax(const Ax &a, int n) { return Ax{min(max(a.i, -1), n - 1), a.w}; }

struct AxS {
  int i;
  float w;
  bool hi;
};
template <bool NANCHK = true>
__device__ __forceinline__ AxS axis_raw_s(float c, float fn) {
  if (NANCHK) c = (c != c) ? 0.f : c;
  const float xb = c * fn - 0.5f;
  const float fl = floorf(xb);
  const float r = xb - fl;
  const float w = NANCHK ? rintf(r * 256.f) * (1.f / 256.f) : frac8_rn(r);
  return AxS{(int)fl, w, r >= 0.5f};
}
template <bool NANCHK = true>
__device__ __forceinline__ AxS axis_cube_s(float p, float hs) {
  float a = p + 1.f;
  if (NANCHK) a = (a != a) ? 0.f : a;
  const float xb = fmaf(a, hs, -0.5f);
  const float fl = floorf(xb);
  const float r = xb - fl;
  const float w = NANCHK ? rintf(r * 256.f) * (1.f / 256.f) : frac8_rn(r);
  return AxS{(int)fl, w, r >= 0.5f};
}

__device__ __forceinline__ void half_taps(const AxS &a, Ax &plus, Ax &minus) {
  const int ip = a.i + (a.hi ? 1 : 0);
  const float wt = a.w + (a.hi ? -0.5f : 0.5f);
  plus = Ax{ip, wt};
  minus = Ax{ip - 1, wt};
}

__device__ __forceinline__ float sqrt_cr(float x) {
  const uint32_t u = __float_as_uint(x);
  if (__builtin_expect(__all(u - 1u >= 0x0f7fffffu), 1)) {
    const float s = __builtin_amdgcn_sqrtf(x);
    const float sm = __uint_as_float(__float_as_uint(s) - 1u), sp = __uint_as_float(__float_as_uint(s) + 1u);
    const float rm = fmaf(-sm, s, x), rp = fmaf(-sp, s, x);
    const float r = (rm <= 0.f) ? sm : s;
    return (rp > 0.f) ? sp : r;
  }
  return sqrtf(x);
}

__device__ __forceinline__ float sqrt_fast(float x) {
  const float s = __builtin_amdgcn_sqrtf(x);
  const float sm = __uint_as_float(__float_as_uint(s) - 1u), sp = __uint_as_float(__float_as_uint(s) + 1u);
  const float rm = fmaf(-sm, s, x), rp = fmaf(-sp, s, x);
  const float r = (rm <= 0.f) ? sm : s;
  return (rp > 0.f) ? sp : r;
}
template <int N>
__device__ __forceinline__ void sqrt_cr_n(const float (&x)[N], float (&out)[N]) {
  bool ok = true;
#pragma unroll
  for (int i = 0; i < N; ++i) ok = ok && (__float_as_uint(x[i]) - 1u >= 0x0f7fffffu);
  if (__builtin_expect(__all(ok), 1)) {
#pragma unroll
    for (int i = 0; i < N; ++i) out[i] = sqrt_fast(x[i]);
  } else {
#pragma unroll
    for (int i = 0; i < N; ++i) out[i] = sqrtf(x[i]);
  }
}

__device__ __forceinline__ float lerp(float a, float b, float w) { return fmaf(w, b - a, a); }

template <bool BIG>
__device__ __forceinline__ float fetch(const DevTex &t, const Ax &ax, const Ax &ay, const Ax &az) {
  const float *b;
  if (BIG) {
    const uint64_t o = ((uint64_t)(az.i + 1) * t.pxy + (uint64_t)(ay.i + 1) * t.px) + (uint64_t)(ax.i + 1);
    b = t.p + o;
  } else {
    const uint32_t o = ((uint32_t)(az.i + 1) * t.pxy + (uint32_t)(ay.i + 1) * t.px) + (uint32_t)(ax.i + 1);
    b = t.p + o;
  }
  const f2a4 r00 = *reinterpret_cast<const f2a4 *>(b);
  const f2a4 r10 = *reinterpret_cast<const f2a4 *>(b + t.px);
  const f2a4 r01 = *reinterpret_cast<const f2a4 *>(b + t.pxy);
  const f2a4 r11 = *reinterpret_cast<const f2a4 *>(b + t.pxy + t.px);
  const float c00 = lerp(r00.x, r00.y, ax.w), c10 = lerp(r10.x, r10.y, ax.w);
  const float c01 = lerp(r01.x, r01.y, ax.w), c11 = lerp(r11.x, r11.y, ax.w);
  const float c0 = lerp(c00, c10, ay.w), c1 = lerp(c01, c11, ay.w);
  return lerp(c0, c1, az.w);
}

struct AxF {
  float fl;
  float w;
};

template <bool FMA = false, bool RN8 = false>
__device__ __forceinline__ AxF axis_lut(float c, float fn) {
  c = __builtin_amdgcn_fmed3f(c, 0.f, 1.f);
  const float xb = FMA ? fmaf(c, fn, -0.5f) : c * fn - 0.5f;
  const float fl = floorf(xb);
  return AxF{fl, RN8 ? weight8_rn(xb, fl) : weight8(xb, fl)};
}

__device__ __forceinline__ float fetch_small(const DevTex &t, const AxF &ax, const AxF &ay, const AxF &az) {
  const uint32_t o = (uint32_t)fmaf(az.fl, t.fpxy4, fmaf(ay.fl, t.fpx4, fmaf(ax.fl, 4.f, t.fbase4)));
  const uint32_t px4 = t.px * 4u, pxy4 = t.pxy * 4u;
  const char *b = reinterpret_cast<const char *>(t.p);
  const f2a4 r00 = *reinterpret_cast<const f2a4 *>(b + o);
  const f2a4 r10 = *reinterpret_cast<const f2a4 *>(b + (o + px4));
  const f2a4 r01 = *reinterpret_cast<const f2a4 *>(b + (o + pxy4));
  const f2a4 r11 = *reinterpret_cast<const f2a4 *>(b + (o + pxy4 + px4));
  const float c00 = lerp(r00.x, r00.y, ax.w), c10 = lerp(r10.x, r10.y, ax.w);
  const float c01 = lerp(r01.x, r01.y, ax.w), c11 = lerp(r11.x, r11.y, ax.w);
  const float c0 = lerp(c00, c10, ay.w), c1 = lerp(c01, c11, ay.w);
  return lerp(c0, c1, az.w);
}
__device__ __forceinline__ void fetch_small2(const DevTex &t, const AxF &ax, const AxF &ay0, const AxF &az0,
                                             const AxF &ay1, const AxF &az1, float &v0, float &v1) {
  const float ox = fmaf(ax.fl, 4.f, t.fbase4);
  const uint32_t o0 = (uint32_t)fmaf(az0.fl, t.fpxy4, fmaf(ay0.fl, t.fpx4, ox));
  const uint32_t o1 = (uint32_t)fmaf(az1.fl, t.fpxy4, fmaf(ay1.fl, t.fpx4, ox));
  const uint32_t px4 = t.px * 4u, pxy4 = t.pxy * 4u;
  const char *b = reinterpret_cast<const char *>(t.p);
  const f2a4 a00 = *reinterpret_cast<const f2a4 *>(b + o0);
  const f2a4 a10 = *reinterpret_cast<const f2a4 *>(b + (o0 + px4));
  const f2a4 a01 = *reinterpret_cast<const f2a4 *>(b + (o0 + pxy4));
  const f2a4 a11 = *reinterpret_cast<const f2a4 *>(b + (o0 + pxy4 + px4));
  const f2a4 b00 = *reinterpret_cast<const f2a4 *>(b + o1);
  const f2a4 b10 = *reinterpret_cast<const f2a4 *>(b + (o1 + px4));
  const f2a4 b01 = *reinterpret_cast<const f2a4 *>(b + (o1 + pxy4));
  const f2a4 b11 = *reinterpret_cast<const f2a4 *>(b + (o1 + pxy4 + px4));
  {
    const float c00 = lerp(a00.x, a00.y, ax.w), c10 = lerp(a10.x, a10.y, ax.w);
    const float c01 = lerp(a01.x, a01.y, ax.w), c11 = lerp(a11.x, a11.y, ax.w);
    v0 = lerp(lerp(c00, c10, ay0.w), lerp(c01, c11, ay0.w), az0.w);
  }
  {
    const float c00 = lerp(b00.x, b00.y, ax.w), c10 = lerp(b10.x, b10.y, ax.w);
    const float c01 = lerp(b01.x, b01.y, ax.w), c11 = lerp(b11.x, b11.y, ax.w);
    v1 = lerp(lerp(c00, c10, ay1.w), lerp(c01, c11, ay1.w), az1.w);
  }
}
#ifndef VR_LUT_ZPAIR
#define VR_LUT_ZPAIR 1
#endif
__device__ __forceinline__ float lerp_zrows(const f4a8 &r0, const f4a8 &r1, const AxF &ax, const AxF &ay,
                                            const AxF &az) {
  const float c00 = lerp(r0.x, r0.z, ax.w), c10 = lerp(r1.x, r1.z, ax.w);
  const float c01 = lerp(r0.y, r0.w, ax.w), c11 = lerp(r1.y, r1.w, ax.w);
  const float c0 = lerp(c00, c10, ay.w), c1 = lerp(c01, c11, ay.w);
  return lerp(c0, c1, az.w);
}
__device__ __forceinline__ float fetch_small_z(const DevTex &t, const AxF &ax, const AxF &ay, const AxF &az) {
  const uint32_t o = (uint32_t)fmaf(az.fl, t.fpxy4, fmaf(ay.fl, t.fpx4, fmaf(ax.fl, 4.f, t.fbase4)));
  const uint32_t o2 = o + o, px8 = t.px * 8u;
  const char *b = reinterpret_cast<const char *>(t.zp);
  const f4a8 r0 = *reinterpret_cast<const f4a8 *>(b + o2);
  const f4a8 r1 = *reinterpret_cast<const f4a8 *>(b + (o2 + px8));
  return lerp_zrows(r0, r1, ax, ay, az);
}
__device__ __forceinline__ void fetch_small2_z(const DevTex &t, const AxF &ax, const AxF &ay0, const AxF &az0,
                                               const AxF &ay1, const AxF &az1, float &v0, float &v1) {
  const float ox = fmaf(ax.fl, 4.f, t.fbase4);
  const uint32_t o0 = (uint32_t)fmaf(az0.fl, t.fpxy4, fmaf(ay0.fl, t.fpx4, ox));
  const uint32_t o1 = (uint32_t)fmaf(az1.fl, t.fpxy4, fmaf(ay1.fl, t.fpx4, ox));
  const uint32_t px8 = t.px * 8u;
  const char *b = reinterpret_cast<const char *>(t.zp);
  const f4a8 a0 = *reinterpret_cast<const f4a8 *>(b + (o0 + o0));
  const f4a8 a1 = *reinterpret_cast<const f4a8 *>(b + (o0 + o0 + px8));
  const f4a8 b0 = *reinterpret_cast<const f4a8 *>(b + (o1 + o1));
  const f4a8 b1 = *reinterpret_cast<const f4a8 *>(b + (o1 + o1 + px8));
  v0 = lerp_zrows(a0, a1, ax, ay0, az0);
  v1 = lerp_zrows(b0, b1, ax, ay1, az1);
}
__device__ __forceinline__ Ax to_ax(const AxF &a) { return Ax{(int)a.fl, a.w}; }

template <bool FMA = false>
__device__ __forceinline__ float lut_light(const DevTex &lut, const AxF &la, float beta, float gamma) {
  if (lut.p == nullptr) return 0.f;
  if (lut.one) {
    const float q = lut.p[0];
    return fmaf(0.5f, q - q, q);
  }
  const AxF lb = axis_lut<FMA>(beta, lut.fny), lg = axis_lut<FMA>(gamma, lut.fnz);
  if (lut.small) return fetch_small(lut, la, lb, lg);
  return fetch<false>(lut, to_ax(la), to_ax(lb), to_ax(lg));
}

struct GvCell {
  float4 a00, b00, a10, b10, a01, b01, a11, b11;
};
template <bool BIG>
__device__ __forceinline__ GvCell gvec_load(const float *gvec, const DevTex &t, uint32_t row8, uint32_t plane8,
                                            const Ax &ax, const Ax &ay, const Ax &az) {
  GvCell q;
  if (VR_GVEC_BRICK) {
    const uint32_t X = (uint32_t)(ax.i + 1), Y = (uint32_t)(ay.i + 1), Z = (uint32_t)(az.i + 1);
    const uint32_t dx = (X & 1u) ? 7u : 1u, dy = (Y & 1u) ? row8 - 2u : 2u, dz = (Z & 1u) ? plane8 - 4u : 4u;
    const uint32_t xy = ((X >> 1) << 3) + (X & 1u) + (Y >> 1) * row8 + ((Y & 1u) << 1) + ((Z & 1u) << 2);
    uint64_t o;
    if (BIG) o = (uint64_t)(Z >> 1) * plane8 + xy;
    else o = (Z >> 1) * plane8 + xy;
    const float4 *b = reinterpret_cast<const float4 *>(gvec) + o;
    q.a00 = b[0], q.b00 = b[dx], q.a10 = b[dy], q.b10 = b[dy + dx];
    q.a01 = b[dz], q.b01 = b[dz + dx], q.a11 = b[dz + dy], q.b11 = b[dz + dy + dx];
  } else {
    uint64_t o;
    if (BIG) o = ((uint64_t)(az.i + 1) * t.pxy + (uint64_t)(ay.i + 1) * t.px) + (uint64_t)(ax.i + 1);
    else o = ((uint32_t)(az.i + 1) * t.pxy + (uint32_t)(ay.i + 1) * t.px) + (uint32_t)(ax.i + 1);
    const float4 *b = reinterpret_cast<const float4 *>(gvec) + o;
    q.a00 = b[0], q.b00 = b[1], q.a10 = b[t.px], q.b10 = b[t.px + 1];
    q.a01 = b[t.pxy], q.b01 = b[t.pxy + 1], q.a11 = b[t.pxy + t.px], q.b11 = b[t.pxy + t.px + 1];
  }
  return q;
}
__device__ __forceinline__ f3 gvec_lerp(const GvCell &q, const Ax &ax, const Ax &ay, const Ax &az) {
  f3 r;
#define VR_TRI(c)                                                                                  \
  {                                                                                                \
    const float c00 = lerp(q.a00.c, q.b00.c, ax.w), c10 = lerp(q.a10.c, q.b10.c, ax.w);            \
    const float c01 = lerp(q.a01.c, q.b01.c, ax.w), c11 = lerp(q.a11.c, q.b11.c, ax.w);            \
    const float c0 = lerp(c00, c10, ay.w), c1 = lerp(c01, c11, ay.w);                              \
    r.c = lerp(c0, c1, az.w);                                                                      \
  }
  VR_TRI(x)
  VR_TRI(y)
  VR_TRI(z)
#undef VR_TRI
  return r;
}
template <bool BIG>
__device__ __forceinline__ f3 fetch_vec(const float *gvec, const DevTex &t, uint32_t row8, uint32_t plane8,
                                        const Ax &ax, const Ax &ay, const Ax &az) {
  return gvec_lerp(gvec_load<BIG>(gvec, t, row8, plane8, ax, ay, az), ax, ay, az);
}

template <bool BIG>
__device__ __forceinline__ float tex3d(const DevTex &t, float x, float y, float z) {
  if (t.p == nullptr) return 0.f;
  if (t.one) {
    const float v = t.p[0];
    return fmaf(0.5f, v - v, v);
  }
  return fetch<BIG>(t, axis(x, t.nx, t.fnx), axis(y, t.ny, t.fny), axis(z, t.nz, t.fnz));
}


#ifndef VR_MIN_WAVES
#define VR_MIN_WAVES 1
#endif

__device__ __forceinline__ bool tile_of_block(const RenderParams &P, int &tx, int &ty) {
  const int b = blockIdx.x;
  const int ntx = (P.part_cols + 15) >> 4, nty = (P.height + 15) >> 4;
  if (P.tile_mode == 0) {
    tx = b % ntx;
    ty = b / ntx;
  } else {
    const int nsx = (ntx + 7) >> 3;
    const int j = b >> 3, s = ((j >> 6) << 3) + (b & 7), w = j & 63;
    tx = (s % nsx) * 8 + (w & 7);
    ty = (s / nsx) * 8 + (w >> 3);
  }
  return tx < ntx && ty < nty;
}

__device__ __forceinline__ bool ray_setup(const RenderParams &P, int x, int y, f3 &o, f3 &d, float &tnear,
                                          float &tfar, int view = 0) {
  const float u = fmaf((float)x / P.fw, 2.f, -1.f);
  const float v = fmaf(((float)y / P.fh) * 2.f, P.ratio, -P.ratio);
  o = view ? mk(P.eye2[0], P.eye2[1], P.eye2[2]) : mk(P.eye[0], P.eye[1], P.eye[2]);
  f3 du;
  du.x = fmaf(P.focal, P.zdir[0], fmaf(v, P.ydir[0], u * P.nx_[0]));
  du.y = fmaf(P.focal, P.zdir[1], fmaf(v, P.ydir[1], u * P.nx_[1]));
  du.z = fmaf(P.focal, P.zdir[2], fmaf(v, P.ydir[2], u * P.nx_[2]));
  const float inv = 1.f / sqrt_cr(dot3(du, du));
  d = mk(du.x * inv, du.y * inv, du.z * inv);
  const f3 bmin = mk(P.bmin[0], P.bmin[1], P.bmin[2]);
  const f3 bmax = mk(-P.bmin[0], -P.bmin[1], -P.bmin[2]);
  const f3 id = mk(1.f / d.x, 1.f / d.y, 1.f / d.z);
  float tmin = ((id.x < 0.f ? bmax.x : bmin.x) - o.x) * id.x;
  float tmax = ((id.x < 0.f ? bmin.x : bmax.x) - o.x) * id.x;
  const float tymin = ((id.y < 0.f ? bmax.y : bmin.y) - o.y) * id.y;
  const float tymax = ((id.y < 0.f ? bmin.y : bmax.y) - o.y) * id.y;
  bool hit = !((tmin > tymax) || (tymin > tmax));
  if (tymin > tmin) tmin = tymin;
  if (tymax < tmax) tmax = tymax;
  const float tzmin = ((id.z < 0.f ? bmax.z : bmin.z) - o.z) * id.z;
  const float tzmax = ((id.z < 0.f ? bmin.z : bmax.z) - o.z) * id.z;
  hit = hit && !((tmin > tzmax) || (tzmin > tmax));
  if (tzmin > tmin) tmin = tzmin;
  if (tzmax < tmax) tmax = tzmax;
  tnear = tmin < 0.f ? 0.f : tmin;
  tfar = tmax;
  return hit;
}

#ifndef VR_ABLATE
#define VR_ABLATE 0
#endif

__device__ __forceinline__ float div_acos_arg(float a, float b) {
  const uint32_t ub = __float_as_uint(b) & 0x7fffffffu;
  if (__builtin_expect(__all(ub - 0x2b800000u <= 0x28000000u), 1)) {
    const float y0 = __builtin_amdgcn_rcpf(b);
    const float y1 = fmaf(fmaf(-b, y0, 1.f), y0, y0);
    const float q0 = a * y1;
    const float q1 = fmaf(fmaf(-b, q0, a), y1, q0);
    return fmaf(fmaf(-b, q1, a), y1, q1);
  }
  return a / b;
}

__device__ __forceinline__ float div_fast(float a, float b) {
  const float y0 = __builtin_amdgcn_rcpf(b);
  const float y1 = fmaf(fmaf(-b, y0, 1.f), y0, y0);
  const float q0 = a * y1;
  const float q1 = fmaf(fmaf(-b, q0, a), y1, q0);
  return fmaf(fmaf(-b, q1, a), y1, q1);
}
__device__ __forceinline__ float div_short(float a, float b) {
  const float y = __builtin_amdgcn_rcpf(b);
  const float q0 = a * y;
  return fmaf(fmaf(-b, q0, a), y, q0);
}
template <int N>
__device__ __forceinline__ void div_acos_n(const float (&a)[N], const float (&b)[N], float (&q)[N]) {
  bool ok = true;
#pragma unroll
  for (int i = 0; i < N; ++i) ok = ok && ((__float_as_uint(b[i]) & 0x7fffffffu) - 0x2b800000u <= 0x28000000u);
  if (__builtin_expect(__all(ok), 1)) {
#pragma unroll
    for (int i = 0; i < N; ++i) q[i] = div_fast(a[i], b[i]);
  } else {
#pragma unroll
    for (int i = 0; i < N; ++i) q[i] = a[i] / b[i];
  }
}

__device__ __forceinline__ float divpi(float x) {
  const float r = 0x1.45f306p-2f;
  const float q = x * r;
  return fmaf(fmaf(-q, VR_PI, x), r, q);
}

#ifndef VR_FAST_ACOS
#define VR_FAST_ACOS 1
#endif
#ifndef VR_ACOS_LITERALS
#define VR_ACOS_LITERALS 1
#endif
#ifndef VR_FAST_NLEN
#define VR_FAST_NLEN 1
#endif
#ifndef VR_FAST_COS
#define VR_FAST_COS 1
#endif
#ifndef VR_FAST_NX
#define VR_FAST_NX 0
#endif
#ifndef VR_FAST_GX
#define VR_FAST_GX 0
#endif
#ifndef VR_FAST_NXQ
#define VR_FAST_NXQ 0
#endif
#ifndef VR_FAST_GXQ
#define VR_FAST_GXQ 0
#endif
#ifndef VR_FAST_HYBQ
#define VR_FAST_HYBQ 0
#endif
#ifndef VR_FAST_HYBRID
#define VR_FAST_HYBRID 0
#endif
#ifndef VR_HYB_TA
#define VR_HYB_TA 0.01f
#endif
#ifndef VR_HYB_TG
#define VR_HYB_TG 0.999f
#endif
#ifndef VR_HYB_TU
#define VR_HYB_TU 2.f
#endif
#ifndef VR_RSQ_NR
#define VR_RSQ_NR 0
#endif
__device__ __forceinline__ float rsq_c(float x) {
  const float y = __builtin_amdgcn_rsqf(x);
#if VR_RSQ_NR
  const float r = fmaf(-(x * y), y, 1.f);
  return fmaf(r * 0.5f, y, y);
#else
  return y;
#endif
}
__device__ __forceinline__ float rcp_sqrt_cr(float x) {
  const uint32_t u = __float_as_uint(x);
  if (__builtin_expect(__all(u == 0u || u - 0x17800000u <= 0x50000000u), 1)) {
    const float r = div_fast(1.f, sqrt_fast(x));
    return u == 0u ? __builtin_inff() : r;
  }
  return 1.f / sqrtf(x);
}
extern "C" __device__ float __ocml_acospi_f32(float);
__device__ __forceinline__ float acospi_q(float q);
#ifndef VR_FAST_CLAMP
#define VR_FAST_CLAMP 1
#endif
__device__ __forceinline__ float acospi_f(float q) {
  if (VR_FAST_CLAMP == 2) q = q < -1.f ? -1.f : q;
  return acospi_q(q);
}
__device__ __forceinline__ float acospi_q(float q) {
#if VR_ABLATE & 2
  return fmaf(q, -0.5f, 0.5f);
#endif
#if VR_FAST_ACOS
  const float t = fabsf(q);
#if VR_ACOS_LITERALS
  float p;
  asm("v_mov_b32 %0, 0x3967ab32\n\t"
      "v_fmaak_f32 %0, %0, %1, 0xbaa77072\n\t"
      "v_fmaak_f32 %0, %0, %1, 0x3b67639e\n\t"
      "v_fmaak_f32 %0, %0, %1, 0xbbd8c4b8\n\t"
      "v_fmaak_f32 %0, %0, %1, 0x3c2a004e\n\t"
      "v_fmaak_f32 %0, %0, %1, 0xbc83f1fe\n\t"
      "v_fmaak_f32 %0, %0, %1, 0x3ce82823\n\t"
      "v_fmaak_f32 %0, %0, %1, 0xbd8be5f3\n\t"
      "v_fmaak_f32 %0, %0, %1, 0x3f000000"
      : "=&v"(p)
      : "v"(t));
#else
  float p = 2.209365193e-04f;
  p = fmaf(p, t, -1.277460018e-03f);
  p = fmaf(p, t, 3.530717921e-03f);
  p = fmaf(p, t, -6.615247577e-03f);
  p = fmaf(p, t, 1.037604921e-02f);
  p = fmaf(p, t, -1.610660180e-02f);
  p = fmaf(p, t, 2.833945118e-02f);
  p = fmaf(p, t, -6.830968708e-02f);
  p = fmaf(p, t, 0.5f);
#endif
  const float r = __builtin_amdgcn_sqrtf(VR_FAST_CLAMP == 1 ? fabsf(1.f - t) : 1.f - t) * p;
  const float sg = __builtin_copysignf(1.f, q);
  return fmaf(sg, r, fmaf(-0.5f, sg, 0.5f));
#else
  return __ocml_acospi_f32(q);
#endif
}

__device__ __attribute__((noinline)) float exp_neg_rn_general(float x) { return (float)exp(-(double)x); }
__device__ __forceinline__ float exp_neg_rn(float x, bool small = false) {
  const float x2 = x * x;
  const float q = fmaf(x, x * (1.f / 24.f) + (-1.f / 6.f), 0.5f);
  float e = 1.f + fmaf(x2, q, -x);
  if (!small && __builtin_expect(!__all(fabsf(x) < 0x1p-7f), 0))
    if (!(fabsf(x) < 0x1p-7f)) e = exp_neg_rn_general(x);
  return e;
}

#ifndef VR_OPACITY_EXP2
#define VR_OPACITY_EXP2 0
#endif
template <bool FAST>
__device__ __forceinline__ float opacity(float a, float tstep, bool small = false) {
#if VR_ABLATE & 8
  return a * tstep;
#elif VR_OPACITY_EXP2
  return 1.f - __builtin_amdgcn_exp2f(-(a * tstep) * 1.44269504088896341f);
#else
  return 1.f - exp_neg_rn(a * tstep, small);
#endif
}

__device__ __forceinline__ DevLight light_at(const RenderParams &P, int i) {
  typedef const __attribute__((address_space(4))) DevLight *cptr;
  const cptr q = (cptr)P.lights + i;
  return DevLight{q->px, q->py, q->pz, q->cr, q->cg, q->cb};
}
__device__ __forceinline__ float voxel0(const float *p) {
  typedef const __attribute__((address_space(4))) float *cptr;
  return ((cptr)p)[0];
}

template <bool TAME, bool XN, bool XG, bool NEED, int NL = 0>
__device__ __forceinline__ void shade_fast(const RenderParams &P, const f3 g, const f3 pos, const f3 o,
                                          const float refl, float &ir, float &ig, float &ib, bool &need,
                                          const DevLight *pre = nullptr) {
  static_assert(NL == 0 || ((NL == 1 || NL == 2) && TAME), "specialised for hoisted lights only");
  const int nl = NL ? NL : P.num_lights;
  float ginv;
  if constexpr (XN) ginv = rcp_sqrt_cr(dot3(g, g));
  else if (VR_FAST_NXQ) ginv = __builtin_amdgcn_rcpf(__builtin_amdgcn_sqrtf(dot3(g, g)));
  else ginv = __builtin_amdgcn_rsqf(dot3(g, g));
  const f3 n = mk(-(g.x * ginv), -(g.y * ginv), -(g.z * ginv));
  const f3 li = mk(o.x - pos.x, o.y - pos.y, o.z - pos.z);
  const float dli = dot3(li, n);
  const f3 lip = mk(fmaf(-dli, n.x, li.x), fmaf(-dli, n.y, li.y), fmaf(-dli, n.z, li.z));
#if VR_FAST_NLEN
  const float rn = 1.f;
#else
  const float rn = rsq_c(dot3(n, n));
#endif
  const float lip2 = dot3(lip, lip), li2 = dot3(li, li);
  const float rlip = XG ? sqrt_cr(lip2) : (VR_FAST_GXQ ? __builtin_amdgcn_sqrtf(lip2) : rsq_c(lip2));
  auto gamma_q = [&](const f3 &lo, const f3 &lop) {
    const float lop2 = dot3(lop, lop);
    float q;
    if constexpr (XG) q = div_acos_arg(dot3(lip, lop), rlip * sqrt_cr(lop2));
    else if (VR_FAST_GXQ) q = div_short(dot3(lip, lop), rlip * __builtin_amdgcn_sqrtf(lop2));
    else q = dot3(lip, lop) * (rlip * rsq_c(lop2));
    if constexpr (NEED) need = need || fabsf(q) > VR_HYB_TG || lop2 < VR_HYB_TA * dot3(lo, lo);
    if constexpr (VR_FAST_HYBQ == 2 && !XG && !NEED) {
      const float aq = fabsf(q);
      if (__builtin_expect(aq > VR_HYB_TG && aq < VR_HYB_TU, 0)) q = dot3(lip, lop) / (sqrtf(lip2) * sqrtf(lop2));
    } else if constexpr (VR_FAST_HYBQ == 1 && !XG && !NEED) {
      const bool nd = fabsf(q) > VR_HYB_TG;
      if (__builtin_expect(__any(nd), 0)) {
        const float qx = div_acos_arg(dot3(lip, lop), sqrt_cr(lip2) * sqrt_cr(lop2));
        if (nd) q = qx;
      }
    }
    return q;
  };
  if constexpr (NEED) need = lip2 < VR_HYB_TA * li2;
  const float alpha_n = acospi_f(dot3(n, li) * (rn * rsq_c(li2)));
  const AxF la = axis_lut<true, TAME>(alpha_n, P.lut.fnx);
  int i = 0;
  if (TAME || (P.lut.p != nullptr && P.lut.small && !P.lut.one)) {
    for (; i + 1 < nl; i += 2) {
      const DevLight L0 = NL == 2 ? pre[0] : ((pre && i == 0) ? pre[0] : light_at(P, i));
      const DevLight L1 = NL == 2 ? pre[1] : ((pre && i == 0) ? pre[1] : light_at(P, i + 1));
      const f3 lo0 = mk(L0.px - pos.x, L0.py - pos.y, L0.pz - pos.z);
      const f3 lo1 = mk(L1.px - pos.x, L1.py - pos.y, L1.pz - pos.z);
      const float dlo0 = dot3(lo0, n), dlo1 = dot3(lo1, n);
      const f3 lop0 = mk(fmaf(-dlo0, n.x, lo0.x), fmaf(-dlo0, n.y, lo0.y), fmaf(-dlo0, n.z, lo0.z));
      const f3 lop1 = mk(fmaf(-dlo1, n.x, lo1.x), fmaf(-dlo1, n.y, lo1.y), fmaf(-dlo1, n.z, lo1.z));
      const float beta0 = acospi_f(dlo0 * (rn * rsq_c(dot3(lo0, lo0))));
      const float gamma0 = acospi_f(gamma_q(lo0, lop0));
      const float beta1 = acospi_f(dlo1 * (rn * rsq_c(dot3(lo1, lo1))));
      const float gamma1 = acospi_f(gamma_q(lo1, lop1));
      float light0, light1;
#if VR_ABLATE & 1
      light0 = beta0 + gamma0 + la.w;
      light1 = beta1 + gamma1 + la.w;
#else
      if (TAME && VR_LUT_ZPAIR)
        fetch_small2_z(P.lut, la, axis_lut<true, TAME>(beta0, P.lut.fny), axis_lut<true, TAME>(gamma0, P.lut.fnz),
                       axis_lut<true, TAME>(beta1, P.lut.fny), axis_lut<true, TAME>(gamma1, P.lut.fnz), light0, light1);
      else
        fetch_small2(P.lut, la, axis_lut<true, TAME>(beta0, P.lut.fny), axis_lut<true, TAME>(gamma0, P.lut.fnz),
                     axis_lut<true, TAME>(beta1, P.lut.fny), axis_lut<true, TAME>(gamma1, P.lut.fnz), light0, light1);
#endif
      const float rl0 = refl * light0;
      ir = fmaf(rl0 * L0.cr, P.color[0], ir);
      ig = fmaf(rl0 * L0.cg, P.color[1], ig);
      ib = fmaf(rl0 * L0.cb, P.color[2], ib);
      const float rl1 = refl * light1;
      ir = fmaf(rl1 * L1.cr, P.color[0], ir);
      ig = fmaf(rl1 * L1.cg, P.color[1], ig);
      ib = fmaf(rl1 * L1.cb, P.color[2], ib);
    }
  }
  if constexpr (!TAME) for (; i + 1 < nl; i += 2) {
    const DevLight L0 = light_at(P, i), L1 = light_at(P, i + 1);
    const f3 lo0 = mk(L0.px - pos.x, L0.py - pos.y, L0.pz - pos.z);
    const f3 lo1 = mk(L1.px - pos.x, L1.py - pos.y, L1.pz - pos.z);
    const float dlo0 = dot3(lo0, n), dlo1 = dot3(lo1, n);
    const f3 lop0 = mk(fmaf(-dlo0, n.x, lo0.x), fmaf(-dlo0, n.y, lo0.y), fmaf(-dlo0, n.z, lo0.z));
    const f3 lop1 = mk(fmaf(-dlo1, n.x, lo1.x), fmaf(-dlo1, n.y, lo1.y), fmaf(-dlo1, n.z, lo1.z));
    const float beta0 = acospi_f(dlo0 * (rn * rsq_c(dot3(lo0, lo0))));
    const float gamma0 = acospi_f(gamma_q(lo0, lop0));
    const float beta1 = acospi_f(dlo1 * (rn * rsq_c(dot3(lo1, lo1))));
    const float gamma1 = acospi_f(gamma_q(lo1, lop1));
    const float light0 = lut_light<true>(P.lut, la, beta0, gamma0);
    const float light1 = lut_light<true>(P.lut, la, beta1, gamma1);
    const float rl0 = refl * light0;
    ir = fmaf(rl0 * L0.cr, P.color[0], ir);
    ig = fmaf(rl0 * L0.cg, P.color[1], ig);
    ib = fmaf(rl0 * L0.cb, P.color[2], ib);
    const float rl1 = refl * light1;
    ir = fmaf(rl1 * L1.cr, P.color[0], ir);
    ig = fmaf(rl1 * L1.cg, P.color[1], ig);
    ib = fmaf(rl1 * L1.cb, P.color[2], ib);
  }
  if (i < nl) {
    const DevLight L = NL == 1 ? pre[0] : light_at(P, i);
    const f3 lo = mk(L.px - pos.x, L.py - pos.y, L.pz - pos.z);
    const float dlo = dot3(lo, n);
    const f3 lop = mk(fmaf(-dlo, n.x, lo.x), fmaf(-dlo, n.y, lo.y), fmaf(-dlo, n.z, lo.z));
    const float beta = acospi_f(dlo * (rn * rsq_c(dot3(lo, lo))));
    const float gamma = acospi_f(gamma_q(lo, lop));
    const float rl = refl * (TAME ? (VR_LUT_ZPAIR ? fetch_small_z(P.lut, la, axis_lut<true, TAME>(beta, P.lut.fny),
                                                                 axis_lut<true, TAME>(gamma, P.lut.fnz))
                                                  : fetch_small(P.lut, la, axis_lut<true, TAME>(beta, P.lut.fny),
                                                                axis_lut<true, TAME>(gamma, P.lut.fnz)))
                                  : lut_light<true>(P.lut, la, beta, gamma));
    ir = fmaf(rl * L.cr, P.color[0], ir);
    ig = fmaf(rl * L.cg, P.color[1], ig);
    ib = fmaf(rl * L.cb, P.color[2], ib);
  }
}

template <bool FAST, bool TAME = false, int NL = 0>
__device__ __forceinline__ void shade_lights(const RenderParams &P, const f3 g, const f3 pos, const f3 o,
                                             const float refl, float &ir, float &ig, float &ib,
                                             const DevLight *pre = nullptr) {
#if !VR_FAST_COS
  if constexpr (FAST) {
    const float ginv = 1.f / sqrt_cr(dot3(g, g));
    const f3 n = mk(-(g.x * ginv), -(g.y * ginv), -(g.z * ginv));
    const f3 li = mk(o.x - pos.x, o.y - pos.y, o.z - pos.z);
    const float dli = dot3(li, n);
    const f3 lip = mk(fmaf(-dli, n.x, li.x), fmaf(-dli, n.y, li.y), fmaf(-dli, n.z, li.z));
    float sq_in[3] = {dot3(n, n), dot3(li, li), dot3(lip, lip)}, sq[3];
    sqrt_cr_n<3>(sq_in, sq);
    const float nlen = sq[0], liplen = sq[2];
    float alpha_n;
    {
      const float num[1] = {dot3(n, li)}, den[1] = {nlen * sq[1]};
      float q[1];
      div_acos_n<1>(num, den, q);
      alpha_n = acospi_q(q[0]);
    }
    const AxF la = axis_lut<true>(alpha_n, P.lut.fnx);
    for (int i = 0; i < P.num_lights; ++i) {
      const DevLight L = light_at(P, i);
      const f3 lo = mk(L.px - pos.x, L.py - pos.y, L.pz - pos.z);
      const float dlo = dot3(lo, n);
      const f3 lop = mk(fmaf(-dlo, n.x, lo.x), fmaf(-dlo, n.y, lo.y), fmaf(-dlo, n.z, lo.z));
      float li_in[2] = {dot3(lo, lo), dot3(lop, lop)}, ln[2];
      sqrt_cr_n<2>(li_in, ln);
      const float num[2] = {dot3(n, lo), dot3(lip, lop)}, den[2] = {nlen * ln[0], liplen * ln[1]};
      float q[2];
      div_acos_n<2>(num, den, q);
      const float rl = refl * lut_light<true>(P.lut, la, acospi_q(q[0]), acospi_q(q[1]));
      ir = fmaf(rl * L.cr, P.color[0], ir);
      ig = fmaf(rl * L.cg, P.color[1], ig);
      ib = fmaf(rl * L.cb, P.color[2], ib);
    }
  } else
#endif
  if constexpr (FAST) {
#if VR_FAST_HYBRID
    bool need = false;
    const float ir0 = ir, ig0 = ig, ib0 = ib;
    shade_fast<TAME, false, false, true>(P, g, pos, o, refl, ir, ig, ib, need);
    if (__any(need)) {
      float er = ir0, eg = ig0, eb = ib0;
      bool unused = false;
      shade_fast<TAME, true, true, false>(P, g, pos, o, refl, er, eg, eb, unused);
      if (need) {
        ir = er;
        ig = eg;
        ib = eb;
      }
    }
#else
    bool unused = false;
    shade_fast<TAME, VR_FAST_NX, VR_FAST_GX, false, NL>(P, g, pos, o, refl, ir, ig, ib, unused, pre);
#endif
  } else {
    const float ginv = 1.f / sqrt_cr(dot3(g, g));
    const f3 n = mk(-(g.x * ginv), -(g.y * ginv), -(g.z * ginv));
    const f3 li = mk(o.x - pos.x, o.y - pos.y, o.z - pos.z);
    const float dli = dot3(li, n);
    const f3 lip = mk(fmaf(-dli, n.x, li.x), fmaf(-dli, n.y, li.y), fmaf(-dli, n.z, li.z));
    float sq_in[3] = {dot3(n, n), dot3(li, li), dot3(lip, lip)}, sq[3];
    sqrt_cr_n<3>(sq_in, sq);
    const float nlen = sq[0], liplen = sq[2];
    float alpha_n;
    {
#if VR_ABLATE & 2
      alpha_n = dot3(n, li) * 0.1f;
#else
      const float num[1] = {dot3(n, li)}, den[1] = {nlen * sq[1]};
      float q[1];
      div_acos_n<1>(num, den, q);
      alpha_n = divpi(acosf(q[0]));
#endif
    }
    const AxF la = axis_lut(alpha_n, P.lut.fnx);
    int i = 0;
    for (; i + 1 < P.num_lights; i += 2) {
      const DevLight L0 = light_at(P, i), L1 = light_at(P, i + 1);
      const f3 lo0 = mk(L0.px - pos.x, L0.py - pos.y, L0.pz - pos.z);
      const f3 lo1 = mk(L1.px - pos.x, L1.py - pos.y, L1.pz - pos.z);
      const float dlo0 = dot3(lo0, n), dlo1 = dot3(lo1, n);
      const f3 lop0 = mk(fmaf(-dlo0, n.x, lo0.x), fmaf(-dlo0, n.y, lo0.y), fmaf(-dlo0, n.z, lo0.z));
      const f3 lop1 = mk(fmaf(-dlo1, n.x, lo1.x), fmaf(-dlo1, n.y, lo1.y), fmaf(-dlo1, n.z, lo1.z));
      float beta0, gamma0, beta1, gamma1;
#if VR_ABLATE & 2
      beta0 = dot3(n, lo0) * 0.01f; gamma0 = dot3(lip, lo0) * 0.01f + liplen;
      beta1 = dot3(n, lo1) * 0.01f; gamma1 = dot3(lip, lo1) * 0.01f + liplen;
#else
      float li_in[4] = {dot3(lo0, lo0), dot3(lop0, lop0), dot3(lo1, lo1), dot3(lop1, lop1)}, ln[4];
      sqrt_cr_n<4>(li_in, ln);
      const float num[4] = {dot3(n, lo0), dot3(lip, lop0), dot3(n, lo1), dot3(lip, lop1)};
      const float den[4] = {nlen * ln[0], liplen * ln[1], nlen * ln[2], liplen * ln[3]};
      float q[4];
      div_acos_n<4>(num, den, q);
      beta0 = divpi(acosf(q[0]));
      gamma0 = divpi(acosf(q[1]));
      beta1 = divpi(acosf(q[2]));
      gamma1 = divpi(acosf(q[3]));
#endif
#if VR_ABLATE & 1
      const float light0 = beta0 + gamma0 + la.w, light1 = beta1 + gamma1 + la.w;
#else
      const float light0 = lut_light(P.lut, la, beta0, gamma0);
      const float light1 = lut_light(P.lut, la, beta1, gamma1);
#endif
      const float rl0 = refl * light0;
      ir = fmaf(rl0 * L0.cr, P.color[0], ir);
      ig = fmaf(rl0 * L0.cg, P.color[1], ig);
      ib = fmaf(rl0 * L0.cb, P.color[2], ib);
      const float rl1 = refl * light1;
      ir = fmaf(rl1 * L1.cr, P.color[0], ir);
      ig = fmaf(rl1 * L1.cg, P.color[1], ig);
      ib = fmaf(rl1 * L1.cb, P.color[2], ib);
    }
    if (i < P.num_lights) {
      const DevLight L = light_at(P, i);
      const f3 lo = mk(L.px - pos.x, L.py - pos.y, L.pz - pos.z);
      const float dlo = dot3(lo, n);
      const f3 lop = mk(fmaf(-dlo, n.x, lo.x), fmaf(-dlo, n.y, lo.y), fmaf(-dlo, n.z, lo.z));
#if VR_ABLATE & 2
      const float beta = dot3(n, lo) * 0.01f, gamma = dot3(lip, lo) * 0.01f + liplen;
#else
      float li_in[2] = {dot3(lo, lo), dot3(lop, lop)}, ln[2];
      sqrt_cr_n<2>(li_in, ln);
      const float num[2] = {dot3(n, lo), dot3(lip, lop)}, den[2] = {nlen * ln[0], liplen * ln[1]};
      float q[2];
      div_acos_n<2>(num, den, q);
      const float beta = divpi(acosf(q[0])), gamma = divpi(acosf(q[1]));
#endif
#if VR_ABLATE & 1
      const float light = beta + gamma + la.w;
#else
      const float light = lut_light(P.lut, la, beta, gamma);
#endif
      const float rl = refl * light;
      ir = fmaf(rl * L.cr, P.color[0], ir);
      ig = fmaf(rl * L.cg, P.color[1], ig);
      ib = fmaf(rl * L.cb, P.color[2], ib);
    }
  }
}

}
```

volume_renderer_amd/csrc/vr_stage.h:

```cpp
#pragma once
#include <hip/hip_runtime.h>
#include <stdint.h>
#include <math.h>
#include <type_traits>

#include "vr_device.h"
#include "vr_sampling.h"

namespace vr {

#ifndef VR_LDS_CAP
#define VR_LDS_CAP 1664
#endif
#ifndef VR_LDS_CAP_MARCH
#define VR_LDS_CAP_MARCH 2040
#endif
#ifndef VR_LDS_CAP_WIDE
#define VR_LDS_CAP_WIDE 2560
#endif
#ifndef VR_STAGE_UNROLL
#define VR_STAGE_UNROLL 4
#endif
#ifndef VR_STAGE_NT
#define VR_STAGE_NT 0
#endif
#ifndef VR_CHUNK
#define VR_CHUNK 32
#endif
#ifndef VR_ATTEMPTS
#define VR_ATTEMPTS 3
#endif

template <int CTRL>
__device__ __forceinline__ int row_ror(int v) {
  return __builtin_amdgcn_mov_dpp(v, CTRL, 0xf, 0xf, false);
}

template <bool MAX>
__device__ __forceinline__ int wave_reduce(int v) {
  int o = row_ror<0x128>(v);
  v = MAX ? max(v, o) : min(v, o);
  o = row_ror<0x124>(v);
  v = MAX ? max(v, o) : min(v, o);
  o = row_ror<0x122>(v);
  v = MAX ? max(v, o) : min(v, o);
  o = row_ror<0x121>(v);
  v = MAX ? max(v, o) : min(v, o);
  const auto p16 = __builtin_amdgcn_permlane16_swap(v, v, false, false);
  v = MAX ? max((int)p16[0], (int)p16[1]) : min((int)p16[0], (int)p16[1]);
  const auto p32 = __builtin_amdgcn_permlane32_swap(v, v, false, false);
  v = MAX ? max((int)p32[0], (int)p32[1]) : min((int)p32[0], (int)p32[1]);
  return __builtin_amdgcn_readfirstlane(v);
}
__device__ __forceinline__ int wave_min(int v) { return wave_reduce<false>(v); }
__device__ __forceinline__ int wave_max(int v) { return wave_reduce<true>(v); }

typedef short vr_s2 __attribute__((ext_vector_type(2)));
__device__ __forceinline__ int pk_min(int a, int b) {
  return __builtin_bit_cast(int, __builtin_elementwise_min(__builtin_bit_cast(vr_s2, a), __builtin_bit_cast(vr_s2, b)));
}
__device__ __forceinline__ int wave_min2(int v) {
  v = pk_min(v, row_ror<0x128>(v));
  v = pk_min(v, row_ror<0x124>(v));
  v = pk_min(v, row_ror<0x122>(v));
  v = pk_min(v, row_ror<0x121>(v));
  const auto p16 = __builtin_amdgcn_permlane16_swap(v, v, false, false);
  v = pk_min((int)p16[0], (int)p16[1]);
  const auto p32 = __builtin_amdgcn_permlane32_swap(v, v, false, false);
  v = pk_min((int)p32[0], (int)p32[1]);
  return __builtin_amdgcn_readfirstlane(v);
}
__device__ __forceinline__ int pk2(int lo16, int hi16) { return (lo16 & 0xffff) | (int)((uint32_t)hi16 << 16); }
__device__ __forceinline__ int pk_lo(int v) { return (int)(short)(v & 0xffff); }
__device__ __forceinline__ int pk_hi(int v) { return v >> 16; }
#ifndef VR_PACKED_BOUNDS
#define VR_PACKED_BOUNDS 1
#endif

#ifndef VR_RELOAD_TEX
#define VR_RELOAD_TEX 0
#endif

#ifndef VR_ODD_PITCH
#define VR_ODD_PITCH 0
#endif

struct Box {
  int rx, ry, rz, ex, ey, ez, px, pxy;
};

__device__ __forceinline__ float lds_tri(const float *L, const Box &B, int a, float wx, float wy, float wz) {
  const float c00 = lerp(L[a], L[a + 1], wx);
  const float c10 = lerp(L[a + B.px], L[a + B.px + 1], wx);
  const float c01 = lerp(L[a + B.pxy], L[a + B.pxy + 1], wx);
  const float c11 = lerp(L[a + B.pxy + B.px], L[a + B.pxy + B.px + 1], wx);
  const float c0 = lerp(c00, c10, wy), c1 = lerp(c01, c11, wy);
  return lerp(c0, c1, wz);
}

struct Cell {
  float c00, c10, c01, c11, c0, c1;
};
__device__ __forceinline__ float lds_tri_cell(const float *L, const Box &B, int a, float wx, float wy, float wz,
                                              Cell &C) {
  C.c00 = lerp(L[a], L[a + 1], wx);
  C.c10 = lerp(L[a + B.px], L[a + B.px + 1], wx);
  C.c01 = lerp(L[a + B.pxy], L[a + B.pxy + 1], wx);
  C.c11 = lerp(L[a + B.pxy + B.px], L[a + B.pxy + B.px + 1], wx);
  C.c0 = lerp(C.c00, C.c10, wy);
  C.c1 = lerp(C.c01, C.c11, wy);
  return lerp(C.c0, C.c1, wz);
}

__device__ __forceinline__ f3 half_grad_lds(const float *L, const Box &B, int ac, const AxS &sx, const AxS &sy,
                                            const AxS &sz, float wx, float wy, float wz, const Cell &C) {
  f3 g;
  {
    const float tx = sx.w + (sx.hi ? -0.5f : 0.5f);
    const int w = ac + (sx.hi ? 0 : -1);
    float m[4], p[4];
#pragma unroll
    for (int r = 0; r < 4; ++r) {
      const int o = w + ((r & 1) ? B.px : 0) + ((r & 2) ? B.pxy : 0);
      const float x0 = L[o], x1 = L[o + 1], x2 = L[o + 2];
      m[r] = lerp(x0, x1, tx);
      p[r] = lerp(x1, x2, tx);
    }
    const float gm = lerp(lerp(m[0], m[1], wy), lerp(m[2], m[3], wy), wz);
    const float gp = lerp(lerp(p[0], p[1], wy), lerp(p[2], p[3], wy), wz);
    g.x = gp - gm;
  }
  {
    const float ty = sy.w + (sy.hi ? -0.5f : 0.5f);
    const int w = ac + (sy.hi ? 2 * B.px : -B.px);
    const float e0 = lerp(L[w], L[w + 1], wx), e1 = lerp(L[w + B.pxy], L[w + B.pxy + 1], wx);
    const float y00 = sy.hi ? C.c00 : e0, y01 = sy.hi ? C.c10 : C.c00, y02 = sy.hi ? e0 : C.c10;
    const float y10 = sy.hi ? C.c01 : e1, y11 = sy.hi ? C.c11 : C.c01, y12 = sy.hi ? e1 : C.c11;
    const float gm = lerp(lerp(y00, y01, ty), lerp(y10, y11, ty), wz);
    const float gp = lerp(lerp(y01, y02, ty), lerp(y11, y12, ty), wz);
    g.y = gp - gm;
  }
  {
    const float tz = sz.w + (sz.hi ? -0.5f : 0.5f);
    const int w = ac + (sz.hi ? 2 * B.pxy : -B.pxy);
    const float q0 = lerp(L[w], L[w + 1], wx), q1 = lerp(L[w + B.px], L[w + B.px + 1], wx);
    const float pe = lerp(q0, q1, wy);
    const float z0 = sz.hi ? C.c0 : pe, z1 = sz.hi ? C.c1 : C.c0, z2 = sz.hi ? pe : C.c1;
    g.z = lerp(z1, z2, tz) - lerp(z0, z1, tz);
  }
  return g;
}

__device__ __forceinline__ int slot_coord(int i, int r) { return (int)((uint32_t)i + 1u - (uint32_t)r); }
__device__ __forceinline__ bool in_box(int l, int e) {
  return (VR_ABLATE & 16) || (unsigned)l < (unsigned)(e - 1);
}

__device__ __forceinline__ DevTex reload(const DevTex &t) {
#if VR_RELOAD_TEX == 1
  typedef const volatile __attribute__((address_space(4))) DevTex *cptr;
  cptr q = (cptr)&t;
  DevTex u;
  u.p = q->p;
  u.nx = q->nx;
  u.ny = q->ny;
  u.nz = q->nz;
  u.px = q->px;
  u.pxy = q->pxy;
  return u;
#elif VR_RELOAD_TEX == 2
  typedef const __attribute__((address_space(4))) DevTex *cptr;
  cptr q = (cptr)&t;
  asm volatile("" : "+s"(q));
  return *q;
#else
  return t;
#endif
}

template <bool BIG>
__device__ __forceinline__ float fetch_at(const DevTex &t, const float *L, const Box &B, bool in, int a,
                                          const Ax &ax, const Ax &ay, const Ax &az) {
  if (in) return lds_tri(L, B, a, ax.w, ay.w, az.w);
  const DevTex u = reload(t);
  return fetch<BIG>(u, clamp_ax(ax, u.nx), clamp_ax(ay, u.ny), clamp_ax(az, u.nz));
}

__device__ __forceinline__ void axis_range(float c0, float c1, float off, int n, int &lo, int &hi, bool &edge) {
  const float cmin = fminf(c0, c1) - off, cmax = fmaxf(c0, c1) + off;
  const int a = (int)floorf(cmin), b = (int)floorf(cmax);
  edge = edge || a < -1 || b > n - 1;
  lo = min(max(a, -1), n - 1) + 1;
  hi = min(max(b, -1), n - 1) + 2;
}

__device__ __forceinline__ bool stage_box_elems(float *L, const DevTex &t, const Box &B, int lane) {
  bool nz = false;
  const uint32_t ex = (uint32_t)B.ex, ey = (uint32_t)B.ey;
  const uint32_t V = ex * ey * (uint32_t)B.ez;
  uint32_t x = (uint32_t)lane % ex;
  uint32_t r = (uint32_t)lane / ex;
  uint32_t y = r % ey, z = r / ey;
  const uint32_t sx = 64u % ex, sr = 64u / ex;
  for (uint32_t q0 = (uint32_t)lane; q0 < V; q0 += 256u) {
    float v[4];
    uint32_t li[4];
#pragma unroll
    for (int j = 0; j < 4; ++j) {
      const uint32_t q = q0 + 64u * j;
      li[j] = z * (uint32_t)B.pxy + y * (uint32_t)B.px + x;
      if (q < V) {
        const uint64_t o = ((uint64_t)(B.rz + z) * t.pxy + (uint64_t)(B.ry + y) * t.px) + (uint64_t)(B.rx + x);
        v[j] = t.p[o];
        nz |= (v[j] != 0.f);
      }
      x += sx;
      y += sr;
      if (x >= ex) {
        x -= ex;
        ++y;
      }
      while (y >= ey) {
        y -= ey;
        ++z;
      }
    }
#pragma unroll
    for (int j = 0; j < 4; ++j) {
      const uint32_t q = q0 + 64u * j;
      if (q < V) L[li[j]] = v[j];
    }
  }
  return __any(nz);
}


#ifndef VR_STAGE_GLDS
#define VR_STAGE_GLDS 0
#endif

template <bool BIG>
__device__ __forceinline__ bool stage_box_glds(float *L, const DevTex &t, const Box &B, int lane) {
  const uint32_t ex = (uint32_t)B.ex, ey = (uint32_t)B.ey;
  const uint32_t V = ex * ey * (uint32_t)B.ez;
  uint32_t x = (uint32_t)lane % ex, r = (uint32_t)lane / ex;
  uint32_t y = r % ey;
  const float *src = t.p + ((uint64_t)(B.rz + r / ey) * t.pxy + (uint64_t)(B.ry + y) * t.px + (uint64_t)(B.rx + x));
  const uint32_t sx = 64u % ex, sr = 64u / ex;
  const int64_t g_step = (int64_t)sx + (int64_t)sr * (int64_t)t.px;
  const int64_t g_row = (int64_t)t.px - (int64_t)ex, g_wrap = (int64_t)t.pxy - (int64_t)ey * (int64_t)t.px;
  __builtin_amdgcn_s_waitcnt(0xC07F);
  for (uint32_t q0 = 0; q0 < V; q0 += 64u) {
    if (q0 + (uint32_t)lane < V)
      __builtin_amdgcn_global_load_lds((const void *)src, (__attribute__((address_space(3))) void *)(L + q0), 4, 0, 0);
    x += sx;
    y += sr;
    src += g_step;
    if (x >= ex) {
      x -= ex;
      ++y;
      src += g_row;
    }
    while (y >= ey) {
      y -= ey;
      src += g_wrap;
    }
  }
  __builtin_amdgcn_s_waitcnt(0x0F70);
  uint32_t acc = 0;
  for (uint32_t q = (uint32_t)lane; q < V; q += 64u) acc |= __float_as_uint(L[q]);
  return __any((acc & 0x7fffffffu) != 0u);
}

template <bool BIG>
__device__ __forceinline__ bool stage_box(float *L, const DevTex &t, const Box &B, int lane) {
  const int ex = B.ex, ey = B.ey;
  if (VR_STAGE_GLDS && B.px == ex && B.pxy == ex * ey &&
      (BIG || (uint64_t)t.pxy * (uint64_t)B.ez * 4u < 0xFFFFFFFFull))
    return stage_box_glds<BIG>(L, t, B, lane);
  if (ex > 64) return stage_box_elems(L, t, B, lane);
  if (!BIG && (uint64_t)t.pxy * (uint64_t)B.ez * 4u >= 0xFFFFFFFFull)
    return stage_box_elems(L, t, B, lane);
  typedef typename std::conditional<BIG, uint64_t, uint32_t>::type off_t;
  const int per = 64 / ex;
  const int rr = lane / ex, xr = lane - rr * ex;
  const int rows = ey * B.ez;
  const int n = rr < per ? (rows - rr + per - 1) / per : 0;
  int y = rr % ey;
  const int z = rr / ey;
  const char *base = reinterpret_cast<const char *>(
      t.p + ((uint64_t)B.rz * t.pxy + (uint64_t)B.ry * t.px + (uint64_t)B.rx));
  off_t g = ((off_t)z * t.pxy + (off_t)y * t.px + (off_t)xr) * 4u;
  const off_t g_row = (off_t)per * t.px * 4u;
  const off_t g_wrap = ((off_t)t.pxy - (off_t)ey * t.px) * 4u;
  int l = z * B.pxy + y * B.px + xr;
  const int l_row = per * B.px;
  const int l_wrap = B.pxy - ey * B.px;
  uint32_t acc = 0;
  for (int k0 = 0; k0 < n; k0 += VR_STAGE_UNROLL) {
    float v[VR_STAGE_UNROLL];
    int li[VR_STAGE_UNROLL];
#pragma unroll
    for (int j = 0; j < VR_STAGE_UNROLL; ++j) {
      li[j] = l;
      if (k0 + j < n) {
        const float *src = reinterpret_cast<const float *>(base + g);
        v[j] = VR_STAGE_NT ? __builtin_nontemporal_load(src) : *src;
      }
      l += l_row;
      g += g_row;
      y += per;
      while (y >= ey) {
        y -= ey;
        g += g_wrap;
        l += l_wrap;
      }
    }
#pragma unroll
    for (int j = 0; j < VR_STAGE_UNROLL; ++j) {
      if (k0 + j < n) {
        L[li[j]] = v[j];
        acc |= __float_as_uint(v[j]);
      }
    }
  }
  return __any((acc & 0x7fffffffu) != 0u);
}

#ifndef VR_PARTIAL
#define VR_PARTIAL 1
#endif

template <int CAP>
__device__ __forceinline__ void plan_chunk(const RenderParams &P, bool alive, const f3 &pos, const f3 &step,
                                           float t, float tfar, int &S, bool &staged, bool &partial, Box &B,
                                           int *vol_out = nullptr, bool *edge_out = nullptr, int s0 = VR_CHUNK) {
  const DevTex &E = P.em;
  const f3 bmin = mk(P.bmin[0], P.bmin[1], P.bmin[2]);
  const f3 bsc = mk(P.bscale[0], P.bscale[1], P.bscale[2]);
  const float tstep = P.tstep;
  S = s0;
  staged = false;
  partial = false;
  B = Box{0, 0, 0, 1, 1, 1, 1, 1};
  for (int attempt = 0;; ++attempt) {
    int lo[3] = {0x3fffffff, 0x3fffffff, 0x3fffffff}, hi[3] = {-0x3fffffff, -0x3fffffff, -0x3fffffff};
    bool edge = false;
    if (alive) {
      const float rem = (tfar - t) / tstep;
      const int s_eff = (rem < (float)S) ? max((int)rem + 2, 1) : S;
      const float k = (float)(s_eff - 1);
      const f3 pe = mk(fmaf(step.x, k, pos.x), fmaf(step.y, k, pos.y), fmaf(step.z, k, pos.z));
      axis_range(((pos.x - bmin.x) * bsc.x) * E.fnx - 0.5f, ((pe.x - bmin.x) * bsc.x) * E.fnx - 0.5f,
                 P.tap_off[0], E.nx, lo[0], hi[0], edge);
      axis_range(((pos.y - bmin.y) * bsc.y) * E.fny - 0.5f, ((pe.y - bmin.y) * bsc.y) * E.fny - 0.5f,
                 P.tap_off[1], E.ny, lo[1], hi[1], edge);
      axis_range(((pos.z - bmin.z) * bsc.z) * E.fnz - 0.5f, ((pe.z - bmin.z) * bsc.z) * E.fnz - 0.5f,
                 P.tap_off[2], E.nz, lo[2], hi[2], edge);
    }
    if (VR_PACKED_BOUNDS && E.nx < 16000 && E.ny < 16000 && E.nz < 16000) {
      const int c = 16383;
      const int a = wave_min2(pk2(min(lo[0], c), min(lo[1], c)));
      const int b = wave_min2(pk2(min(lo[2], c), min(-hi[0], c)));
      const int d = wave_min2(pk2(min(-hi[1], c), min(-hi[2], c)));
      B.rx = pk_lo(a);
      B.ry = pk_hi(a);
      B.rz = pk_lo(b);
      B.ex = -pk_hi(b) - B.rx + 1;
      B.ey = -pk_lo(d) - B.ry + 1;
      B.ez = -pk_hi(d) - B.rz + 1;
    } else {
      B.rx = wave_min(lo[0]);
      B.ry = wave_min(lo[1]);
      B.rz = wave_min(lo[2]);
      B.ex = wave_max(hi[0]) - B.rx + 1;
      B.ey = wave_max(hi[1]) - B.ry + 1;
      B.ez = wave_max(hi[2]) - B.rz + 1;
    }
    B.px = VR_ODD_PITCH == 1 ? (B.ex | 1) : B.ex;
    B.pxy = VR_ODD_PITCH == 1 ? ((B.px * B.ey) | 1) : B.px * B.ey;
    if (vol_out) *vol_out = B.pxy * B.ez;
    if (B.ex <= 0 || B.ey <= 0 || B.ez <= 0) return;
    if (B.pxy * B.ez <= CAP) {
      if (VR_ODD_PITCH == 2) {
        const int px = B.ex | 1, pxy = (px * B.ey) | 1;
        if (pxy * B.ez <= CAP) {
          B.px = px;
          B.pxy = pxy;
        }
      }
      staged = true;
      if (edge_out) *edge_out = __any(edge);
      return;
    }
    if (S <= (VR_CHUNK >> (VR_ATTEMPTS - 1))) break;
    S >>= 1;
  }
#if VR_PARTIAL
  int e[3] = {B.ex, B.ey, B.ez}, r[3] = {B.rx, B.ry, B.rz};
  while (e[0] * e[1] * e[2] > CAP) {
    const int a = (e[0] >= e[1] && e[0] >= e[2]) ? 0 : (e[1] >= e[2] ? 1 : 2);
    if (e[a] <= 2) break;
    r[a] += e[a] & 1;
    --e[a];
  }
  B.rx = r[0]; B.ry = r[1]; B.rz = r[2];
  B.ex = e[0]; B.ey = e[1]; B.ez = e[2];
  B.px = B.ex;
  B.pxy = B.ex * B.ey;
  if (B.pxy * B.ez <= CAP) {
    staged = true;
    partial = true;
    return;
  }
#endif
  S >>= 1;
}

typedef const __attribute__((address_space(4))) RenderParams *KParams;
__device__ __forceinline__ KParams kparams_fresh(KParams kp) {
  asm volatile("" : "+s"(kp));
  return kp;
}

__device__ __forceinline__ int probe_run(const RenderParams &P, KParams kp0, bool alive, const f3 &pos,
                                         const f3 &step, float t, float tfar, int L, int lane) {
  const KParams kp = kparams_fresh(kp0);
  const DevTex &E = P.em;
  const f3 bmin = mk(P.bmin[0], P.bmin[1], P.bmin[2]);
  const f3 bsc = mk(P.bscale[0], P.bscale[1], P.bscale[2]);
  int lo[3] = {0x3fffffff, 0x3fffffff, 0x3fffffff}, hi[3] = {-0x3fffffff, -0x3fffffff, -0x3fffffff};
  bool edge = false;
  if (alive) {
    const float rem = (tfar - t) / P.tstep;
    const int s_eff = (rem < (float)L) ? max((int)rem + 2, 1) : L;
    const float k = (float)(s_eff - 1);
    const f3 pe = mk(fmaf(step.x, k, pos.x), fmaf(step.y, k, pos.y), fmaf(step.z, k, pos.z));
    axis_range(((pos.x - bmin.x) * bsc.x) * E.fnx - 0.5f, ((pe.x - bmin.x) * bsc.x) * E.fnx - 0.5f,
               kp->probe_off[0], E.nx, lo[0], hi[0], edge);
    axis_range(((pos.y - bmin.y) * bsc.y) * E.fny - 0.5f, ((pe.y - bmin.y) * bsc.y) * E.fny - 0.5f,
               kp->probe_off[1], E.ny, lo[1], hi[1], edge);
    axis_range(((pos.z - bmin.z) * bsc.z) * E.fnz - 0.5f, ((pe.z - bmin.z) * bsc.z) * E.fnz - 0.5f,
               kp->probe_off[2], E.nz, lo[2], hi[2], edge);
  }
  const int c = 16383;
  const int a = wave_min2(pk2(min(lo[0] >> VR_OCC_LOG, c), min(lo[1] >> VR_OCC_LOG, c)));
  const int b = wave_min2(pk2(min(lo[2] >> VR_OCC_LOG, c), min(-(hi[0] >> VR_OCC_LOG), c)));
  const int d = wave_min2(pk2(min(-(hi[1] >> VR_OCC_LOG), c), min(-(hi[2] >> VR_OCC_LOG), c)));
// ... 160 lines not shown
```

Before: 89.06 Mrays/s.

## Precompute LUT byte-offset scales, fold LDS addressing, and mask-driven march loop

Several micro-optimisations at once. The host now precomputes doubled LUT stride/base constants so the z-pair LUT fetches skip a shift. LDS cell addressing is folded into a single byte address built with mad_i24 and scalar operands, and the acos polynomial's leading constant is hoisted out of the per-angle code. The per-chunk sample loop for K=2/4 is rewritten to track alive/mine lanes as wave ballot masks instead of per-lane branches, and wave index is made scalar. It also adds a test env override for max_steps. The inline asm and mask bookkeeping add complexity and some correctness risk.

```diff
diff --git a/volume_renderer_amd/csrc/vr_capi.hip b/volume_renderer_amd/csrc/vr_capi.hip
--- a/volume_renderer_amd/csrc/vr_capi.hip
+++ b/volume_renderer_amd/csrc/vr_capi.hip
@@ -687,6 +687,10 @@
   P.gy = dev_tex(g_tex.bind[T_DY]);
   P.gz = dev_tex(g_tex.bind[T_DZ]);
   P.lut = dev_tex(g_tex.bind[T_LIGHT]);
+  P.lutz_fpx8 = 2.f * P.lut.fpx4;
+  P.lutz_fpxy8 = 2.f * P.lut.fpxy4;
+  P.lutz_fbase8 = 2.f * P.lut.fbase4;
+  P.lutz_px8 = 8u * P.lut.px;
   P.num_lights = (int32_t)g_tex.lights.size();
   P.lights = nullptr;
   F.mode = P.num_lights == 0 ? 0 : (g_tex.grad_method == G_LOOKUP ? 2 : 1);
@@ -762,6 +766,10 @@
                                        (double)bmax[2] * bmax[2]));
   const double cap = 2.0 * diag / (double)P.tstep + 64.0;
   P.max_steps = (finite && cap < 2.0e9) ? (int32_t)cap : 2000000000;
+  if (const char *ev = test_env("VR_MAX_STEPS")) {
+    const long v = std::strtol(ev, nullptr, 10);
+    if (v > 0 && v < (long)P.max_steps) P.max_steps = (int32_t)v;
+  }
   F.degenerate = !finite;
   return VR_OK;
 }
diff --git a/volume_renderer_amd/csrc/vr_device.h b/volume_renderer_amd/csrc/vr_device.h
--- a/volume_renderer_amd/csrc/vr_device.h
+++ b/volume_renderer_amd/csrc/vr_device.h
@@ -53,6 +53,7 @@
   int32_t tap_half;
   float cube_hs[3];
   int32_t num_lights;
+  float lutz_fpx8;
   const DevLight *lights;
   DevTex em, ab, re, gem, gx, gy, gz, lut;
   const float *gvec;
@@ -77,15 +78,18 @@
   int32_t views;
   int32_t pair_shift;
   uint32_t view_blocks;
+  float lutz_fpxy8;
   const uint32_t *wg_order;
   uint32_t *wg_cost;
   uint32_t *wg_start;
   uint32_t sched_blocks;
   uint32_t sched_full;
   uint32_t prio_blocks;
+  float lutz_fbase8;
   const uint8_t *occ;
   uint32_t occ_bx, occ_bxy;
   float probe_off[3];
+  uint32_t lutz_px8;
   unsigned long long *steps;
   float slab_z0, slab_z1, slab_margin;
   int32_t slab_pk0, slab_pk1, slab_dir;
diff --git a/volume_renderer_amd/csrc/vr_march.hip b/volume_renderer_amd/csrc/vr_march.hip
--- a/volume_renderer_amd/csrc/vr_march.hip
+++ b/volume_renderer_amd/csrc/vr_march.hip
@@ -153,7 +153,7 @@
 #define VR_PROBE_MIN (2 * VR_CHUNK)
 #endif
 
-template <int MODE, bool AB_ALIAS, bool SHARE2, bool BIG, bool NANCHK, int NL = 0>
+template <int MODE, bool AB_ALIAS, bool SHARE2, bool BIG, bool NANCHK, int NL = 0, bool WHOLE_CT = false>
 __device__ __forceinline__ void sample_at(const RenderParams &P, const float *L, const Box &B, bool staged, bool whole,
                                           const f3 pos, const f3 o, float &r, float &gg, float &b, float &alpha,
                                           bool &shaded, float rv = 0.f, const DevLight *pre = nullptr) {
@@ -185,12 +185,27 @@
     ay = axis_raw<NANCHK>(ps.y, E.fny);
     az = axis_raw<NANCHK>(ps.z, E.fnz);
   }
-  const int lx = slot_coord(ax.i, B.rx), ly = slot_coord(ay.i, B.ry), lz = slot_coord(az.i, B.rz);
+  constexpr bool FOLD =
+      WHOLE_CT && VR_MARCH_FAST && MODE == 1 && SHARE2 && VR_MERGED_BOUNDS && VR_WHOLE_BOX && !VR_CHECK_WHOLE;
+  const int lx = FOLD ? 0 : slot_coord(ax.i, B.rx), ly = FOLD ? 0 : slot_coord(ay.i, B.ry),
+            lz = FOLD ? 0 : slot_coord(az.i, B.rz);
 #define inx in_box(lx, B.ex)
 #define iny in_box(ly, B.ey)
 #define inz in_box(lz, B.ez)
   const int ayz = lz * B.pxy + ly * B.px;
   const int ac = ayz + lx;
+  lds_cptr cc;
+  if constexpr (FOLD) {
+    uint32_t kfold = __builtin_amdgcn_readfirstlane(lds_addr(L)) +
+                     4u * (uint32_t)((1 - B.rz) * B.pxy + (1 - B.ry) * B.px + (1 - B.rx));
+    asm("" : "+s"(kfold));
+    uint32_t a4 = ((uint32_t)ax.i << 2) + kfold;
+    asm("v_mad_i32_i24 %0, %1, %2, %0" : "+v"(a4) : "v"(ay.i), "s"(4 * B.px));
+    asm("v_mad_i32_i24 %0, %1, %2, %0" : "+v"(a4) : "v"(az.i), "s"(4 * B.pxy));
+    cc = (lds_cptr)a4;
+  } else {
+    cc = lds_cell(L, ac);
+  }
   Cell C;
   float em_s;
   bool full = false;
@@ -212,8 +227,8 @@
     }
   }
   if constexpr (HALF_TAPS) {
-    if (full) em_s = lds_tri_cell(L, B, ac, ax.w, ay.w, az.w, C);
-    else if (staged && inx && iny && inz) em_s = lds_tri_cell(L, B, ac, ax.w, ay.w, az.w, C);
+    if (full) em_s = lds_tri_cell(cc, B, ax.w, ay.w, az.w, C);
+    else if (staged && inx && iny && inz) em_s = lds_tri_cell(cc, B, ax.w, ay.w, az.w, C);
     else {
       const DevTex U = reload(E);
       em_s = fetch<BIG>(U, clamp_ax(ax, U.nx), clamp_ax(ay, U.ny), clamp_ax(az, U.nz));
@@ -239,7 +254,7 @@
                (full || __all(staged && (unsigned)(lx + (sx.hi ? 1 : 0) - 1) < (unsigned)(B.ex - 2) &&
                      (unsigned)(ly + (sy.hi ? 1 : 0) - 1) < (unsigned)(B.ey - 2) &&
                      (unsigned)(lz + (sz.hi ? 1 : 0) - 1) < (unsigned)(B.ez - 2)))) {
-      g = half_grad_lds(L, B, ac, sx, sy, sz, ax.w, ay.w, az.w, C);
+      g = half_grad_lds(cc, B, sx, sy, sz, ax.w, ay.w, az.w, C);
     } else if (HALF_TAPS && (HALF_ONLY || P.tap_half)) {
       const bool syz = staged && iny && inz, sxz = staged && inx && inz, sxy = staged && inx && iny;
       Ax p, m;
@@ -343,6 +358,20 @@
   }
 }
 
+template <int K>
+__device__ __forceinline__ uint64_t group_or_mask(uint64_t m) {
+  static_assert(K == 2 || K == 4, "lane groups of 2 or 4");
+  if constexpr (K == 2) {
+    const uint64_t x = (m | (m >> 1)) & 0x5555555555555555ull;
+    return x | (x << 1);
+  } else {
+    uint64_t x = m | (m >> 1);
+    x = (x | (x >> 2)) & 0x1111111111111111ull;
+    x |= x << 1;
+    return x | (x << 2);
+  }
+}
+
 template <int K, int I = 0>
 __device__ __forceinline__ int group_max_i(int v, int acc) {
   if constexpr (K == 1 || I == K) {
@@ -356,10 +385,10 @@
 #define VR_ZERO_FILL 1
 #endif
 template <int K, int I, bool ZF = false>
-__device__ __forceinline__ void composite_group(const RenderParams &P, Ray &R, float exf, float r, float gg, float b,
-                                                float alpha, float thr) {
+__device__ __forceinline__ void composite_group(const RenderParams &P, Ray &R, bool &alive, float exf, float r, float gg,
+                                                float b, float alpha, float thr) {
   if constexpr (K == 2 && ZF && I < K) {
-    if (R.alive) {
+    if (alive) {
       const float om = 1.f - R.sa;
       if constexpr (I == 0)
         asm("s_nop 1\n\t"
@@ -377,21 +406,21 @@
             "v_fmac_f32_dpp %3, %7, %8 quad_perm:[1,1,3,3] row_mask:0xf bank_mask:0xf"
             : "+v"(R.sr), "+v"(R.sg), "+v"(R.sb), "+v"(R.sa)
             : "v"(r), "v"(gg), "v"(b), "v"(alpha), "v"(om));
-      if (R.sa > thr) R.alive = false;
-    }
-    composite_group<K, I + 1, ZF>(P, R, exf, r, gg, b, alpha, thr);
+      if (R.sa > thr) alive = false;
+    }
+    composite_group<K, I + 1, ZF>(P, R, alive, exf, r, gg, b, alpha, thr);
   } else if constexpr (I < K) {
     const float ri = group_lane<K, I>(r), gi = group_lane<K, I>(gg), bi = group_lane<K, I>(b),
                 ai = group_lane<K, I>(alpha);
-    if ((ZF || group_lane<K, I>(exf) != 0.f) && R.alive) {
+    if ((ZF || group_lane<K, I>(exf) != 0.f) && alive) {
       const float om = 1.f - R.sa;
       R.sr = fmaf(om, ri, R.sr);
       R.sg = fmaf(om, gi, R.sg);
       R.sb = fmaf(om, bi, R.sb);
       R.sa = fmaf(om, ai, R.sa);
-      if (R.sa > thr) R.alive = false;
-    }
-    composite_group<K, I + 1, ZF>(P, R, exf, r, gg, b, alpha, thr);
+      if (R.sa > thr) alive = false;
+    }
+    composite_group<K, I + 1, ZF>(P, R, alive, exf, r, gg, b, alpha, thr);
   }
 }
 
@@ -602,6 +631,30 @@
     } else {
       auto samples = [&](auto wc) {
       constexpr bool WC = decltype(wc)::value;
+      if constexpr (!NANCHK && !SLAB && !BIG && (K == 2 || K == 4)) {
+        const uint64_t am0 = __ballot(R.alive), mine0 = __ballot(R.mine);
+        uint64_t am = am0, mm = am0 & mine0;
+        for (int k = 0, Su = __builtin_amdgcn_readfirstlane(S); k < Su && am != 0ull; k += K) {
+          if (__builtin_amdgcn_inverse_ballot_w64(am)) {
+            float r = 0.f, gg = 0.f, b = 0.f, alpha = 0.f;
+            bool shaded = false;
+            if (__builtin_amdgcn_inverse_ballot_w64(mm))
+              sample_at<MODE, AB_ALIAS, SHARE2, BIG, NANCHK, NL, WC>(P, L, B, staged, WC || (!VR_WHOLE_SPLIT && whole),
+                                                                 R.pos, R.o, r, gg, b, alpha, shaded, rv, pre);
+            if (COUNT) {
+              ++C.iter;
+              C.lit += (MODE != 0 && __any(shaded)) ? 1u : 0u;
+            }
+            bool go = true, mine = true;
+            composite_group<K, 0, VR_ZERO_FILL>(P, R, go, 1.f, r, gg, b, alpha, thr);
+            advance_k<K>(P, mine, R.nsteps, R.t, R.tfar, R.pos, R.step, cap);
+          }
+          mm &= am & __ballot(R.nsteps < cap) & __ballot(!(R.t > R.tfar));
+          am &= __ballot(!(R.sa > thr)) & group_or_mask<K>(mm);
+        }
+        R.alive = __builtin_amdgcn_inverse_ballot_w64(am);
+        R.mine = __builtin_amdgcn_inverse_ballot_w64(mm | (mine0 & ~am0));
+      } else
       for (int k = 0, Su = __builtin_amdgcn_readfirstlane(S); k < Su; k += K) {
         if (!__any(R.alive)) break;
         if (!R.alive) continue;
@@ -614,14 +667,14 @@
         }
         bool shaded = false;
         if (take) {
-          sample_at<MODE, AB_ALIAS, SHARE2, BIG, NANCHK, NL>(P, L, B, staged, WC || (!VR_WHOLE_SPLIT && whole), R.pos,
-                                                         R.o, r, gg, b, alpha, shaded, rv, pre);
+          sample_at<MODE, AB_ALIAS, SHARE2, BIG, NANCHK, NL, WC>(P, L, B, staged, WC || (!VR_WHOLE_SPLIT && whole),
+                                                             R.pos, R.o, r, gg, b, alpha, shaded, rv, pre);
         }
         if (COUNT) {
           ++C.iter;
           C.lit += (MODE != 0 && __any(shaded)) ? 1u : 0u;
         }
-        composite_group<K, 0, VR_ZERO_FILL && !NANCHK && !SLAB>(P, R, ex ? 1.f : 0.f, r, gg, b, alpha, thr);
+        composite_group<K, 0, VR_ZERO_FILL && !NANCHK && !SLAB>(P, R, R.alive, ex ? 1.f : 0.f, r, gg, b, alpha, thr);
         if (SLAB && !inside) {
           if (R.alive && group_any<K>(R.mine && !ex)) {
             float t = R.t;
@@ -692,7 +745,7 @@
 __global__ __launch_bounds__(64 * VR_WG_WAVES, march_min_eu(CAP, SCHED)) void march_kernel(const RenderParams P) {
   using TS = TileShape<K>;
   __shared__ float lds[VR_WG_WAVES][CAP];
-  const int lane = threadIdx.x & 63, wave = threadIdx.x >> 6;
+  const int lane = threadIdx.x & 63, wave = __builtin_amdgcn_readfirstlane(threadIdx.x >> 6);
   float *L = lds[wave];
   constexpr bool ORDERED = SCHED >= 1 && SCHED <= 3;
   constexpr bool TIMED = SCHED == 1 || SCHED == 2;
diff --git a/volume_renderer_amd/csrc/vr_sampling.h b/volume_renderer_amd/csrc/vr_sampling.h
--- a/volume_renderer_amd/csrc/vr_sampling.h
+++ b/volume_renderer_amd/csrc/vr_sampling.h
@@ -197,25 +197,27 @@
   const float c0 = lerp(c00, c10, ay.w), c1 = lerp(c01, c11, ay.w);
   return lerp(c0, c1, az.w);
 }
-__device__ __forceinline__ float fetch_small_z(const DevTex &t, const AxF &ax, const AxF &ay, const AxF &az) {
-  const uint32_t o = (uint32_t)fmaf(az.fl, t.fpxy4, fmaf(ay.fl, t.fpx4, fmaf(ax.fl, 4.f, t.fbase4)));
-  const uint32_t o2 = o + o, px8 = t.px * 8u;
-  const char *b = reinterpret_cast<const char *>(t.zp);
+__device__ __forceinline__ uint32_t lutz_px8(const RenderParams &P) { return P.lutz_px8; }
+__device__ __forceinline__ float fetch_small_z(const RenderParams &P, const AxF &ax, const AxF &ay, const AxF &az) {
+  const uint32_t o2 =
+      (uint32_t)fmaf(az.fl, P.lutz_fpxy8, fmaf(ay.fl, P.lutz_fpx8, fmaf(ax.fl, 8.f, P.lutz_fbase8)));
+  const uint32_t px8 = lutz_px8(P);
+  const char *b = reinterpret_cast<const char *>(P.lut.zp);
   const f4a8 r0 = *reinterpret_cast<const f4a8 *>(b + o2);
   const f4a8 r1 = *reinterpret_cast<const f4a8 *>(b + (o2 + px8));
   return lerp_zrows(r0, r1, ax, ay, az);
 }
-__device__ __forceinline__ void fetch_small2_z(const DevTex &t, const AxF &ax, const AxF &ay0, const AxF &az0,
+__device__ __forceinline__ void fetch_small2_z(const RenderParams &P, const AxF &ax, const AxF &ay0, const AxF &az0,
                                                const AxF &ay1, const AxF &az1, float &v0, float &v1) {
-  const float ox = fmaf(ax.fl, 4.f, t.fbase4);
-  const uint32_t o0 = (uint32_t)fmaf(az0.fl, t.fpxy4, fmaf(ay0.fl, t.fpx4, ox));
-  const uint32_t o1 = (uint32_t)fmaf(az1.fl, t.fpxy4, fmaf(ay1.fl, t.fpx4, ox));
-  const uint32_t px8 = t.px * 8u;
-  const char *b = reinterpret_cast<const char *>(t.zp);
-  const f4a8 a0 = *reinterpret_cast<const f4a8 *>(b + (o0 + o0));
-  const f4a8 a1 = *reinterpret_cast<const f4a8 *>(b + (o0 + o0 + px8));
-  const f4a8 b0 = *reinterpret_cast<const f4a8 *>(b + (o1 + o1));
-  const f4a8 b1 = *reinterpret_cast<const f4a8 *>(b + (o1 + o1 + px8));
+  const float ox = fmaf(ax.fl, 8.f, P.lutz_fbase8);
+  const uint32_t o0 = (uint32_t)fmaf(az0.fl, P.lutz_fpxy8, fmaf(ay0.fl, P.lutz_fpx8, ox));
+  const uint32_t o1 = (uint32_t)fmaf(az1.fl, P.lutz_fpxy8, fmaf(ay1.fl, P.lutz_fpx8, ox));
+  const uint32_t px8 = lutz_px8(P);
+  const char *b = reinterpret_cast<const char *>(P.lut.zp);
+  const f4a8 a0 = *reinterpret_cast<const f4a8 *>(b + o0);
+  const f4a8 a1 = *reinterpret_cast<const f4a8 *>(b + (o0 + px8));
+  const f4a8 b0 = *reinterpret_cast<const f4a8 *>(b + o1);
+  const f4a8 b1 = *reinterpret_cast<const f4a8 *>(b + (o1 + px8));
   v0 = lerp_zrows(a0, a1, ax, ay0, az0);
   v1 = lerp_zrows(b0, b1, ax, ay1, az1);
 }
@@ -454,11 +456,26 @@
 #ifndef VR_FAST_CLAMP
 #define VR_FAST_CLAMP 1
 #endif
-__device__ __forceinline__ float acospi_f(float q) {
+__device__ __forceinline__ float acospi_c0(float dep) {
+  float c;
+  asm("v_mov_b32 %0, 0x3967ab32" : "=v"(c) : "v"(dep));
+  return c;
+}
+__device__ __forceinline__ float acospi_q(float q, float c0);
+__device__ __forceinline__ float acospi_f(float q, float c0) {
   if (VR_FAST_CLAMP == 2) q = q < -1.f ? -1.f : q;
-  return acospi_q(q);
+  return acospi_q(q, c0);
 }
 __device__ __forceinline__ float acospi_q(float q) {
+#if VR_FAST_ACOS && VR_ACOS_LITERALS
+  float c0;
+  asm("v_mov_b32 %0, 0x3967ab32" : "=v"(c0));
+  return acospi_q(q, c0);
+#else
+  return acospi_q(q, 2.209365193e-04f);
+#endif
+}
+__device__ __forceinline__ float acospi_q(float q, float c0) {
 #if VR_ABLATE & 2
   return fmaf(q, -0.5f, 0.5f);
 #endif
@@ -466,8 +483,7 @@
   const float t = fabsf(q);
 #if VR_ACOS_LITERALS
   float p;
-  asm("v_mov_b32 %0, 0x3967ab32\n\t"
-      "v_fmaak_f32 %0, %0, %1, 0xbaa77072\n\t"
+  asm("v_fmaak_f32 %0, %2, %1, 0xbaa77072\n\t"
       "v_fmaak_f32 %0, %0, %1, 0x3b67639e\n\t"
       "v_fmaak_f32 %0, %0, %1, 0xbbd8c4b8\n\t"
       "v_fmaak_f32 %0, %0, %1, 0x3c2a004e\n\t"
@@ -476,9 +492,9 @@
       "v_fmaak_f32 %0, %0, %1, 0xbd8be5f3\n\t"
       "v_fmaak_f32 %0, %0, %1, 0x3f000000"
       : "=&v"(p)
-      : "v"(t));
-#else
-  float p = 2.209365193e-04f;
+      : "v"(t), "v"(c0));
+#else
+  float p = c0;
   p = fmaf(p, t, -1.277460018e-03f);
   p = fmaf(p, t, 3.530717921e-03f);
   p = fmaf(p, t, -6.615247577e-03f);
@@ -536,6 +552,12 @@
                                           const DevLight *pre = nullptr) {
   static_assert(NL == 0 || ((NL == 1 || NL == 2) && TAME), "specialised for hoisted lights only");
   const int nl = NL ? NL : P.num_lights;
+#if VR_FAST_ACOS && VR_ACOS_LITERALS
+  const float c0 = acospi_c0(g.x);
+#else
+  const float c0 = 2.209365193e-04f;
+#endif
+  auto ang = [&](float q) { return acospi_f(q, c0); };
   float ginv;
   if constexpr (XN) ginv = rcp_sqrt_cr(dot3(g, g));
   else if (VR_FAST_NXQ) ginv = __builtin_amdgcn_rcpf(__builtin_amdgcn_sqrtf(dot3(g, g)));
@@ -571,7 +593,7 @@
     return q;
   };
   if constexpr (NEED) need = lip2 < VR_HYB_TA * li2;
-  const float alpha_n = acospi_f(dot3(n, li) * (rn * rsq_c(li2)));
+  const float alpha_n = ang(dot3(n, li) * (rn * rsq_c(li2)));
   const AxF la = axis_lut<true, TAME>(alpha_n, P.lut.fnx);
   int i = 0;
   if (TAME || (P.lut.p != nullptr && P.lut.small && !P.lut.one)) {
@@ -583,17 +605,17 @@
       const float dlo0 = dot3(lo0, n), dlo1 = dot3(lo1, n);
       const f3 lop0 = mk(fmaf(-dlo0, n.x, lo0.x), fmaf(-dlo0, n.y, lo0.y), fmaf(-dlo0, n.z, lo0.z));
       const f3 lop1 = mk(fmaf(-dlo1, n.x, lo1.x), fmaf(-dlo1, n.y, lo1.y), fmaf(-dlo1, n.z, lo1.z));
-      const float beta0 = acospi_f(dlo0 * (rn * rsq_c(dot3(lo0, lo0))));
-      const float gamma0 = acospi_f(gamma_q(lo0, lop0));
-      const float beta1 = acospi_f(dlo1 * (rn * rsq_c(dot3(lo1, lo1))));
-      const float gamma1 = acospi_f(gamma_q(lo1, lop1));
+      const float beta0 = ang(dlo0 * (rn * rsq_c(dot3(lo0, lo0))));
+      const float gamma0 = ang(gamma_q(lo0, lop0));
+      const float beta1 = ang(dlo1 * (rn * rsq_c(dot3(lo1, lo1))));
+      const float gamma1 = ang(gamma_q(lo1, lop1));
       float light0, light1;
 #if VR_ABLATE & 1
       light0 = beta0 + gamma0 + la.w;
       light1 = beta1 + gamma1 + la.w;
 #else
       if (TAME && VR_LUT_ZPAIR)
-        fetch_small2_z(P.lut, la, axis_lut<true, TAME>(beta0, P.lut.fny), axis_lut<true, TAME>(gamma0, P.lut.fnz),
+        fetch_small2_z(P, la, axis_lut<true, TAME>(beta0, P.lut.fny), axis_lut<true, TAME>(gamma0, P.lut.fnz),
                        axis_lut<true, TAME>(beta1, P.lut.fny), axis_lut<true, TAME>(gamma1, P.lut.fnz), light0, light1);
       else
         fetch_small2(P.lut, la, axis_lut<true, TAME>(beta0, P.lut.fny), axis_lut<true, TAME>(gamma0, P.lut.fnz),
@@ -616,10 +638,10 @@
     const float dlo0 = dot3(lo0, n), dlo1 = dot3(lo1, n);
     const f3 lop0 = mk(fmaf(-dlo0, n.x, lo0.x), fmaf(-dlo0, n.y, lo0.y), fmaf(-dlo0, n.z, lo0.z));
     const f3 lop1 = mk(fmaf(-dlo1, n.x, lo1.x), fmaf(-dlo1, n.y, lo1.y), fmaf(-dlo1, n.z, lo1.z));
-    const float beta0 = acospi_f(dlo0 * (rn * rsq_c(dot3(lo0, lo0))));
-    const float gamma0 = acospi_f(gamma_q(lo0, lop0));
-    const float beta1 = acospi_f(dlo1 * (rn * rsq_c(dot3(lo1, lo1))));
-    const float gamma1 = acospi_f(gamma_q(lo1, lop1));
+    const float beta0 = ang(dlo0 * (rn * rsq_c(dot3(lo0, lo0))));
+    const float gamma0 = ang(gamma_q(lo0, lop0));
+    const float beta1 = ang(dlo1 * (rn * rsq_c(dot3(lo1, lo1))));
+    const float gamma1 = ang(gamma_q(lo1, lop1));
     const float light0 = lut_light<true>(P.lut, la, beta0, gamma0);
     const float light1 = lut_light<true>(P.lut, la, beta1, gamma1);
     const float rl0 = refl * light0;
@@ -636,9 +658,9 @@
     const f3 lo = mk(L.px - pos.x, L.py - pos.y, L.pz - pos.z);
     const float dlo = dot3(lo, n);
     const f3 lop = mk(fmaf(-dlo, n.x, lo.x), fmaf(-dlo, n.y, lo.y), fmaf(-dlo, n.z, lo.z));
-    const float beta = acospi_f(dlo * (rn * rsq_c(dot3(lo, lo))));
-    const float gamma = acospi_f(gamma_q(lo, lop));
-    const float rl = refl * (TAME ? (VR_LUT_ZPAIR ? fetch_small_z(P.lut, la, axis_lut<true, TAME>(beta, P.lut.fny),
+    const float beta = ang(dlo * (rn * rsq_c(dot3(lo, lo))));
+    const float gamma = ang(gamma_q(lo, lop));
+    const float rl = refl * (TAME ? (VR_LUT_ZPAIR ? fetch_small_z(P, la, axis_lut<true, TAME>(beta, P.lut.fny),
                                                                  axis_lut<true, TAME>(gamma, P.lut.fnz))
                                                   : fetch_small(P.lut, la, axis_lut<true, TAME>(beta, P.lut.fny),
                                                                 axis_lut<true, TAME>(gamma, P.lut.fnz)))
diff --git a/volume_renderer_amd/csrc/vr_stage.h b/volume_renderer_amd/csrc/vr_stage.h
--- a/volume_renderer_amd/csrc/vr_stage.h
+++ b/volume_renderer_amd/csrc/vr_stage.h
@@ -101,28 +101,46 @@
 struct Cell {
   float c00, c10, c01, c11, c0, c1;
 };
-__device__ __forceinline__ float lds_tri_cell(const float *L, const Box &B, int a, float wx, float wy, float wz,
-                                              Cell &C) {
-  C.c00 = lerp(L[a], L[a + 1], wx);
-  C.c10 = lerp(L[a + B.px], L[a + B.px + 1], wx);
-  C.c01 = lerp(L[a + B.pxy], L[a + B.pxy + 1], wx);
-  C.c11 = lerp(L[a + B.pxy + B.px], L[a + B.pxy + B.px + 1], wx);
+typedef const __attribute__((address_space(3))) char *lds_cptr;
+__device__ __forceinline__ uint32_t lds_addr(const float *L) {
+  return (uint32_t)(uintptr_t)(const __attribute__((address_space(3))) float *)L;
+}
+__device__ __forceinline__ lds_cptr lds_cell(const float *L, int a) {
+  return (lds_cptr)((const __attribute__((address_space(3))) float *)L + a);
+}
+__device__ __forceinline__ float lds_f(lds_cptr c, int byte) {
+  return *reinterpret_cast<const __attribute__((address_space(3))) float *>(c + byte);
+}
+__device__ __forceinline__ float lds_tri_cell(lds_cptr c, const Box &B, float wx, float wy, float wz, Cell &C) {
+  const int px4 = B.px * 4, pxy4 = B.pxy * 4;
+  C.c00 = lerp(lds_f(c, 0), lds_f(c, 4), wx);
+  C.c10 = lerp(lds_f(c, px4), lds_f(c, px4 + 4), wx);
+  C.c01 = lerp(lds_f(c, pxy4), lds_f(c, pxy4 + 4), wx);
+  C.c11 = lerp(lds_f(c, pxy4 + px4), lds_f(c, pxy4 + px4 + 4), wx);
   C.c0 = lerp(C.c00, C.c10, wy);
   C.c1 = lerp(C.c01, C.c11, wy);
   return lerp(C.c0, C.c1, wz);
 }
 
-__device__ __forceinline__ f3 half_grad_lds(const float *L, const Box &B, int ac, const AxS &sx, const AxS &sy,
-                                            const AxS &sz, float wx, float wy, float wz, const Cell &C) {
+__device__ __forceinline__ int tap_row(bool hi) {
+  int j = hi ? 2 : -1;
+  asm("" : "+v"(j));
+  return j;
+}
+
+__device__ __forceinline__ f3 half_grad_lds(lds_cptr cc, const Box &B, const AxS &sx, const AxS &sy, const AxS &sz,
+                                            float wx, float wy, float wz, const Cell &C) {
   f3 g;
+  auto at = [&](lds_cptr c, int byte) { return lds_f(c, byte); };
+  const int px4 = B.px * 4, pxy4 = B.pxy * 4;
   {
     const float tx = sx.w + (sx.hi ? -0.5f : 0.5f);
-    const int w = ac + (sx.hi ? 0 : -1);
+    const lds_cptr w = cc + (sx.hi ? 0 : -4);
     float m[4], p[4];
 #pragma unroll
     for (int r = 0; r < 4; ++r) {
-      const int o = w + ((r & 1) ? B.px : 0) + ((r & 2) ? B.pxy : 0);
-      const float x0 = L[o], x1 = L[o + 1], x2 = L[o + 2];
+      const int o = ((r & 1) ? px4 : 0) + ((r & 2) ? pxy4 : 0);
+      const float x0 = at(w, o), x1 = at(w, o + 4), x2 = at(w, o + 8);
       m[r] = lerp(x0, x1, tx);
       p[r] = lerp(x1, x2, tx);
     }
@@ -132,8 +150,8 @@
   }
   {
     const float ty = sy.w + (sy.hi ? -0.5f : 0.5f);
-    const int w = ac + (sy.hi ? 2 * B.px : -B.px);
-    const float e0 = lerp(L[w], L[w + 1], wx), e1 = lerp(L[w + B.pxy], L[w + B.pxy + 1], wx);
+    const lds_cptr w = cc + __mul24(tap_row(sy.hi), px4);
+    const float e0 = lerp(at(w, 0), at(w, 4), wx), e1 = lerp(at(w, pxy4), at(w, pxy4 + 4), wx);
     const float y00 = sy.hi ? C.c00 : e0, y01 = sy.hi ? C.c10 : C.c00, y02 = sy.hi ? e0 : C.c10;
     const float y10 = sy.hi ? C.c01 : e1, y11 = sy.hi ? C.c11 : C.c01, y12 = sy.hi ? e1 : C.c11;
     const float gm = lerp(lerp(y00, y01, ty), lerp(y10, y11, ty), wz);
@@ -142,8 +160,8 @@
   }
   {
     const float tz = sz.w + (sz.hi ? -0.5f : 0.5f);
-    const int w = ac + (sz.hi ? 2 * B.pxy : -B.pxy);
-    const float q0 = lerp(L[w], L[w + 1], wx), q1 = lerp(L[w + B.px], L[w + B.px + 1], wx);
+    const lds_cptr w = cc + __mul24(tap_row(sz.hi), pxy4);
+    const float q0 = lerp(at(w, 0), at(w, 4), wx), q1 = lerp(at(w, px4), at(w, px4 + 4), wx);
     const float pe = lerp(q0, q1, wy);
     const float z0 = sz.hi ? C.c0 : pe, z1 = sz.hi ? C.c1 : C.c0, z2 = sz.hi ? pe : C.c1;
     g.z = lerp(z1, z2, tz) - lerp(z0, z1, tz);
```

Result: faster. 92.25 Mrays/s, median of 6 (+3.6%).
